# MCG-NKU/E2FGVI

Hardware: AMD Instinct MI355X
Metric: inpainted frames/sec at 432x240 T=10 (higher is better)
Workload: dtype f32; 1 GPU; BASELINE.json configs[1]: e2fgvi 432x240 T=10 l_t=10, 1 clip(s) per GPU per forward (1 in the job), random-init weights, torch.rand frames + box mask (SURVEY.md 8d); clips_per_gpu=1, precision=fp32, kernel_selection=e2fgvi_amd/tile_table.py (checked in, deterministic: ops.py), hip_graph=True, forwards_in_flight=2

## Files before the change

### e2fgvi_amd/build.py

```python
import os
import subprocess
import sys
from concurrent.futures import ThreadPoolExecutor

HERE = os.path.dirname(os.path.abspath(__file__))
CSRC = os.path.join(HERE, "csrc")
LIB = os.path.join(CSRC, "libe2fgvi_hip.so")
FLAGS = ["--offload-arch=gfx950", "-O3", "-std=c++17", "-fPIC", "-ffp-contract=fast"]
NOPK = ["-Xclang", "-target-feature", "-Xclang", "-packed-fp32-ops"]
UNITS = [("error.hip", "error.o", []), ("conv.hip", "conv.o", []), ("conv.hip", "conv_nopk.o", NOPK + ["-DE2_NOPK_VARIANT"]),
         ("conv_bf16x.hip", "conv_bf16x.o", NOPK), ("conv_wino.hip", "conv_wino.o", NOPK), ("conv_wino.hip", "conv_wino_x3.o", NOPK + ["-DE2_WINO_X3=1"]), ("conv_wino4.hip", "conv_wino4.o", NOPK), ("conv_tail.hip", "conv_tail.o", NOPK),
         ("mdcn.hip", "mdcn.o", NOPK), ("attention.hip", "attention.o", []),
         ("attention_bf16.hip", "attention_bf16.o", NOPK), ("attention_x3.hip", "attention_x3.o", NOPK), ("misc.hip", "misc.o", NOPK),
         ("video.hip", "video.o", NOPK), ("metrics.hip", "metrics.o", NOPK)]
NOPK_OBJECTS = ("conv_nopk.o", "conv_bf16x.o", "conv_wino.o", "conv_wino4.o", "conv_wino_x3.o", "conv_tail.o", "mdcn.o", "attention_bf16.o", "attention_x3.o", "misc.o", "video.o", "metrics.o")
OBJDUMP = "/opt/rocm/lib/llvm/bin/llvm-objdump"


def _hipcc():
    for c in (os.environ.get("HIPCC"), "/opt/rocm/bin/hipcc"):
        if c and os.path.exists(c):
            return c
    return "hipcc"


def _stale(out, deps):
    return (not os.path.exists(out)) or any(os.path.getmtime(d) > os.path.getmtime(out) for d in deps)


def build(force=False, verbose=False, nopk_all=False, lib=None, tag=None, defines=()):
    hipcc = _hipcc()
    if tag:
        nopk_all = False
    objdir = os.path.join(CSRC, ("build_" + tag) if tag else ("build_nopk" if nopk_all else "build"))
    os.makedirs(objdir, exist_ok=True)
    out = lib or (os.path.join(CSRC, "libe2fgvi_hip_%s.so" % tag) if tag else
                  os.path.join(CSRC, "libe2fgvi_hip_nopk.so") if nopk_all else LIB)
    headers = [os.path.join(CSRC, "common.h"), os.path.join(HERE, "..", "include", "e2fgvi_hip.h"), os.path.abspath(__file__)]
    jobs = []
    for src, obj, extra in UNITS:
        sp, op = os.path.join(CSRC, src), os.path.join(objdir, obj)
        if nopk_all and not any(f == "-packed-fp32-ops" for f in extra):
            extra = extra + NOPK
        if force or _stale(op, [sp] + headers):
            jobs.append([hipcc] + FLAGS + extra + list(defines) + ["-c", sp, "-o", op])

    def run(cmd):
        if verbose:
            print(" ".join(cmd), flush=True)
        subprocess.check_call(cmd)

    with ThreadPoolExecutor(max_workers=min(4, max(1, len(jobs)))) as ex:
        list(ex.map(run, jobs))
    objs = [os.path.join(objdir, obj) for _, obj, _ in UNITS]
    if force or jobs or _stale(out, objs):
        run([hipcc, "--offload-arch=gfx950", "-shared", "-fPIC", "-o", out] + objs)
    if jobs:
        verify_isa(objdir)
        if not nopk_all:
            verify_wino_waits(objdir)
            verify_exit_reuse(objdir)
            verify_no_scratch(objdir)
    return out


def build_variant(tag, *defines):
    return build(tag=tag, defines=defines)


def device_isa(obj):
    import shutil
    import tempfile
    d = tempfile.mkdtemp(prefix="e2isa")
    try:
        local = os.path.join(d, os.path.basename(obj))
        shutil.copy(obj, local)
        subprocess.run([OBJDUMP, "--offloading", os.path.basename(obj)], cwd=d, check=True, stdout=subprocess.DEVNULL,
                       stderr=subprocess.DEVNULL)
        dev = [f for f in os.listdir(d) if "gfx950" in f]
        if not dev:
            return ""
        return subprocess.run([OBJDUMP, "-d", os.path.join(d, dev[0])], check=True, capture_output=True, text=True).stdout
    finally:
        shutil.rmtree(d, ignore_errors=True)


def verify_isa(objdir=None):
    import re
    objdir = objdir or os.path.join(CSRC, "build")
    if not os.path.exists(OBJDUMP):
        return
    for obj in NOPK_OBJECTS:
        isa = device_isa(os.path.join(objdir, obj))
        bad = re.findall(r"v_pk_(?:mul|add|fma)_f32", isa)
        if bad or not isa:
            raise RuntimeError("%s: %s" % (obj, "%d packed-fp32 instructions in a unit that must have none" % len(bad) if isa
                                           else "no gfx950 code object found"))


def verify_no_scratch(objdir=None, obj="conv_bf16x.o", marker="ELb0ELi2ELb1EEE"):
    import re
    import shutil
    import tempfile
    objdir = objdir or os.path.join(CSRC, "build")
    readelf = os.path.join(os.path.dirname(OBJDUMP), "llvm-readelf")
    if not (os.path.exists(OBJDUMP) and os.path.exists(readelf)):
        return 0
    d = tempfile.mkdtemp(prefix="e2elf")
    try:
        shutil.copy(os.path.join(objdir, obj), os.path.join(d, obj))
        subprocess.run([OBJDUMP, "--offloading", obj], cwd=d, check=True, stdout=subprocess.DEVNULL, stderr=subprocess.DEVNULL)
        dev = [f for f in os.listdir(d) if "gfx950" in f]
        notes = subprocess.run([readelf, "--notes", os.path.join(d, dev[0])], check=True, capture_output=True, text=True).stdout if dev else ""
    finally:
        shutil.rmtree(d, ignore_errors=True)
    found = 0
    for block in notes.split("  - .agpr_count")[1:]:
        name = re.search(r"\.name:\s+(\S+)", block)
        if not name or marker not in name.group(1):
            continue
        found += 1
        priv = int(re.search(r"\.private_segment_fixed_size:\s+(\d+)", block).group(1))
        spill = int(re.search(r"\.vgpr_spill_count:\s+(\d+)", block).group(1))
        if priv or spill:
            raise RuntimeError("%s: %s: private segment %d bytes, %d spilled VGPRs in a ping-pong kernel" % (obj, name.group(1)[:70], priv, spill))
    if not found:
        raise RuntimeError("verify_no_scratch: no ping-pong instantiation found in %s (mangled-name marker changed?)" % obj)
    return found


def _kernels(isa):
    import re
    out, cur = {}, None
    for line in isa.splitlines():
        m = re.match(r"^[0-9a-f]+ <([^>]+)>:", line)
        if m:
            cur = out.setdefault(m.group(1), [])
            continue
        m = re.match(r"^\s+(\S+)\s*(.*?)\s*//\s*([0-9A-Fa-f]+):", line)
        if m and cur is not None:
            cur.append((int(m.group(3), 16), m.group(1), m.group(2)))
    return out


def check_kernel_waits(obj, name, ins):
    import re
    vmem = re.compile(r"^(buffer|global|flat|scratch)_(load|store|atomic)")
    marks = [i for i in range(len(ins) - 1) if ins[i][1] == "s_waitcnt" and ins[i + 1][1] == "s_waitcnt"
             and ins[i][2] == ins[i + 1][2] and "vmcnt" in ins[i][2]]
    if not marks:
        return 0
    addr_to_idx = {a: i for i, (a, _, _) in enumerate(ins)}
    spans = []
    for i, (a, mn, ops_) in enumerate(ins):
        if mn.startswith("s_cbranch") or mn == "s_branch":
            try:
                off = int(ops_.split()[0])
            except (ValueError, IndexError):
                continue
            if off >= 32768:
                off -= 65536
            tgt = a + 4 + 4 * off
            if off < 0 and tgt in addr_to_idx:
                spans.append((addr_to_idx[tgt], i))
    loops = 0
    rolling = "conv_wino_x3w_kernel" in name
    for lo, hi in spans:
        inner = [m for m in marks if lo <= m <= hi]
        if not inner or any(lo <= l2 and h2 <= hi and (l2, h2) != (lo, hi) and any(l2 <= m <= h2 for m in inner)
                            for l2, h2 in spans):
            continue
        loops += 1
        if rolling:
            counts = [int(re.search(r"vmcnt\((\d+)\)", ins[m][2]).group(1)) for m in inner]
            for a, b in zip(inner, inner[1:]):
                if any(vmem.match(ins[k][1]) for k in range(a + 2, b)):
                    raise RuntimeError("%s: %s: vector-memory instruction between the group waits at 0x%x and 0x%x"
                                       % (obj, name[:60], ins[a][0], ins[b][0]))
            g = counts[0] - counts[1] if len(counts) > 1 else counts[0]
            if counts[-1] != 0 or g <= 0 or any(c != counts[0] - j * g for j, c in enumerate(counts)):
                raise RuntimeError("%s: %s: group waits %s are not (P-1) G, ..., G, 0" % (obj, name[:60], counts))
            tail = [k for k in list(range(inner[-1] + 2, hi + 1)) + list(range(lo, inner[0])) if vmem.match(ins[k][1])]
            planes = tail[-(counts[0] + g):]
            if len(planes) != counts[0] + g or any(ins[k][1] != "buffer_load_dwordx4" or " lds" in ins[k][2] for k in planes):
                raise RuntimeError("%s: %s: the %d vector-memory instructions in front of the group waits are not the plane "
                                   "loads" % (obj, name[:60], counts[0] + g))
            continue
        for j, m in enumerate(inner):
            n = int(re.search(r"vmcnt\((\d+)\)", ins[m][2]).group(1))
            if j:
                rng = range(inner[j - 1] + 2, m)
            else:
                rng = list(range(inner[-1] + 2, hi + 1)) + list(range(lo, m))
            cnt = sum(1 for k in rng if vmem.match(ins[k][1]))
            if cnt != n:
                raise RuntimeError("%s: %s: explicit s_waitcnt vmcnt(%d) at 0x%x follows %d vector-memory instructions "
                                   "since the previous explicit wait" % (obj, name[:60], n, ins[m][0], cnt))
    return loops


def verify_wino_waits(objdir=None, objects=("conv_wino.o", "conv_wino_x3.o", "conv_wino4.o")):
    objdir = objdir or os.path.join(CSRC, "build")
    if not os.path.exists(OBJDUMP):
        return 0
    loops = 0
    for obj in objects:
        for name, ins in _kernels(device_isa(os.path.join(objdir, obj))).items():
            loops += check_kernel_waits(obj, name, ins)
    if not loops:
        raise RuntimeError("verify_wino_waits: no K loop with marked waits found (disassembly format changed?)")
    return loops


def _vregs(text):
    import re
    r = set()
    for m in re.finditer(r"\bv\[(\d+):(\d+)\]", text):
        r.update(range(int(m.group(1)), int(m.group(2)) + 1))
    for m in re.finditer(r"\bv(\d+)\b", text):
        r.add(int(m.group(1)))
    return r


def _successors(ins, at):
    succ = []
    for i, (a, m, o) in enumerate(ins):
        if m in ("s_endpgm", "s_endpgm_saved"):
            succ.append(())
        elif m == "s_branch" or m.startswith("s_cbranch"):
            off = int(o.split()[0])
            off -= 65536 if off > 32767 else 0
            tgt = at.get(a + 4 + 4 * off)
            if tgt is None:
                raise RuntimeError("branch at 0x%x leaves the kernel" % a)
            succ.append((tgt,) if m == "s_branch" else (tgt, i + 1))
        elif m.startswith("s_setpc") or m.startswith("s_swappc"):
            raise RuntimeError("indirect jump at 0x%x: control flow cannot be followed" % a)
        else:
            succ.append((i + 1,) if i + 1 < len(ins) else ())
    return succ


def check_exit_reuse(obj, name, ins, min_mfma=8):
    import re
    at = {a: i for i, (a, _, _) in enumerate(ins)}
    succ = _successors(ins, at)
    is_mfma = [("mfma" in m) for _, m, _ in ins]
    breg = set()
    for (_, m, o), f in zip(ins, is_mfma):
        if f:
            breg |= _vregs([x.strip() for x in o.split(",")][2])
    wregs = set()
    for _, m, o in ins:
        if re.match(r"buffer_load_dword", m) and not o.rstrip().endswith(" lds"):
            d = _vregs(o.split(",")[0])
            if d & breg:
                wregs |= d
    if not wregs:
        return 0
    n = len(ins)
    index, low, comp = [-1] * n, [0] * n, [-1] * n
    stack, onstack, counter, ncomp = [], [False] * n, 0, 0
    for root in range(n):
        if index[root] >= 0:
            continue
        work = [(root, 0)]
        while work:
            v, pi = work.pop()
            if pi == 0:
                index[v] = low[v] = counter
                counter += 1
                stack.append(v)
                onstack[v] = True
            recurse = False
            for j in range(pi, len(succ[v])):
                w = succ[v][j]
                if index[w] < 0:
                    work.append((v, j + 1))
                    work.append((w, 0))
                    recurse = True
                    break
                if onstack[w]:
                    low[v] = min(low[v], index[w])
            if recurse:
                continue
            if low[v] == index[v]:
                while True:
                    w = stack.pop()
                    onstack[w] = False
                    comp[w] = ncomp
                    if w == v:
                        break
                ncomp += 1
            if work:
                u = work[-1][0]
                low[u] = min(low[u], low[v])
    members = {}
    for k in range(n):
        members.setdefault(comp[k], []).append(k)
    loops = [m for m in members.values() if len(m) > 1 and sum(1 for k in m if is_mfma[k]) >= min_mfma]
    inside = [False] * n
    for m in loops:
        for k in m:
            inside[k] = True
    edges = 0
    for m in loops:
        mine = set(m)
        starts = set()
        for k in m:
            for t in succ[k]:
                if t not in mine:
                    starts.add(t)
        for st in sorted(starts):
            edges += 1
            seen, todo = set(), [(st, False)]
            while todo:
                k, dead = todo.pop()
                if (k, dead) in seen:
                    continue
                seen.add((k, dead))
                a, m, o = ins[k]
                if m == "s_waitcnt" and "vmcnt(0)" in o:
                    continue
                if m.startswith("s_endpgm") or (inside[k] and not dead):
                    raise RuntimeError("%s: %s: the path from the K-loop exit at 0x%x reaches 0x%x (%s) without an s_waitcnt vmcnt(0): "
                                       "weight loads may still be in flight" % (obj, name[:60], ins[st][0], a,
                                                                                "another K loop" if inside[k] else m))
                if not dead and not m.startswith("s_") and _vregs(o) & wregs:
                    raise RuntimeError("%s: %s: 0x%x %s %s touches a register of a weight load that may still be in flight behind the "
                                       "K loop left at 0x%x (no vmcnt(0) yet)" % (obj, name[:60], a, m, o, ins[st][0]))
                flip = m == "s_andn2_saveexec_b64" or (m == "s_xor_b64" and o.startswith("exec"))
                if flip and not dead:
                    dead = True
                elif m in ("s_or_b64", "s_mov_b64") and o.startswith("exec"):
                    dead = False
                nxt = succ[k]
                if dead and m == "s_cbranch_execz":
                    nxt = nxt[:1]
                elif dead and m == "s_cbranch_execnz":
                    nxt = nxt[1:]
                todo.extend((t, dead) for t in nxt)
    return edges


EXIT_REUSE_OBJECTS = ("conv_wino.o", "conv_wino_x3.o", "conv_wino4.o")


def verify_exit_reuse(objdir=None, objects=EXIT_REUSE_OBJECTS):
    objdir = objdir or os.path.join(CSRC, "build")
    if not os.path.exists(OBJDUMP):
        return 0
    n = 0
    for obj in objects:
        for name, ins in _kernels(device_isa(os.path.join(objdir, obj))).items():
            if "conv_wino" not in name or "pack_" in name:
                continue
            k = check_exit_reuse(obj, name, ins)
            if not k:
                raise RuntimeError("verify_exit_reuse: no K-loop exit found in %s: %s (disassembly format changed?)" % (obj, name[:60]))
            n += k
    if not n:
        raise RuntimeError("verify_exit_reuse: no Winograd kernel found")
    return n


if __name__ == "__main__":
    print(build(force="--force" in sys.argv, verbose=True, nopk_all="--nopk-all" in sys.argv))
```

### e2fgvi_amd/csrc/conv_wino4.hip

```cpp
#include "common.h"
#include <utility>

#ifndef E2_CLAIM_AFTER_LOOP
#define E2_CLAIM_AFTER_LOOP(r) asm volatile("" : "+v"(r))
#endif

namespace {

struct W4Params {
    const float* src[E2FGVI_MAX_SRC];
    int ld[E2FGVI_MAX_SRC];
    int coff[E2FGVI_MAX_SRC];
    int cpg[E2FGVI_MAX_SRC];
    unsigned src_bytes[E2FGVI_MAX_SRC];
    int nsrc;
    int N, H, W;
    int Cout, Cout_g, Npad;
    int blocksY, blocksX, tilesN, nblk;
    int nchunks;
    unsigned wgroup_bytes;
    long long wgroup_elems;
    const float* w;
    const float* bias;
    const float* res;
    int res_ld, res_coff;
    float* dst;
    int dst_ld, dst_coff;
    int act;
    float slope;
    int vec_store;
};

__host__ __device__ constexpr float bt4(int r, int c) {
    return r == 0   ? (c == 0 ? 4.f : c == 2 ? -5.f : c == 4 ? 1.f : 0.f)
           : r == 1 ? (c == 1 ? -4.f : c == 2 ? -4.f : c == 3 ? 1.f : c == 4 ? 1.f : 0.f)
           : r == 2 ? (c == 1 ? 4.f : c == 2 ? -4.f : c == 3 ? -1.f : c == 4 ? 1.f : 0.f)
           : r == 3 ? (c == 1 ? -2.f : c == 2 ? -1.f : c == 3 ? 2.f : c == 4 ? 1.f : 0.f)
           : r == 4 ? (c == 1 ? 2.f : c == 2 ? -1.f : c == 3 ? -2.f : c == 4 ? 1.f : 0.f)
                    : (c == 1 ? 4.f : c == 3 ? -5.f : c == 5 ? 1.f : 0.f);
}
__host__ __device__ constexpr float bt2(int r, int c) {
    return r == 0   ? (c == 0 ? 1.f : c == 2 ? -1.f : 0.f)
           : r == 1 ? (c == 1 ? 1.f : c == 2 ? 1.f : 0.f)
           : r == 2 ? (c == 1 ? -1.f : c == 2 ? 1.f : 0.f)
                    : (c == 1 ? 1.f : c == 3 ? -1.f : 0.f);
}
__host__ __device__ constexpr float at4(int r, int c) {
    return r == 0   ? (c < 5 ? 1.f : 0.f)
           : r == 1 ? (c == 1 ? 1.f : c == 2 ? -1.f : c == 3 ? 2.f : c == 4 ? -2.f : 0.f)
           : r == 2 ? (c == 1 ? 1.f : c == 2 ? 1.f : c == 3 ? 4.f : c == 4 ? 4.f : 0.f)
                    : (c == 1 ? 1.f : c == 2 ? -1.f : c == 3 ? 8.f : c == 4 ? -8.f : c == 5 ? 1.f : 0.f);
}
__host__ __device__ constexpr float at2(int r, int c) {
    return r == 0 ? (c < 3 ? 1.f : 0.f) : (c == 1 ? 1.f : c == 2 ? -1.f : c == 3 ? -1.f : 0.f);
}
__host__ __device__ constexpr float g4(int r, int c) {
    return r == 0   ? (c == 0 ? 0.25f : 0.f)
           : r == 1 ? (-1.f / 6.f)
           : r == 2 ? (c == 1 ? 1.f / 6.f : -1.f / 6.f)
           : r == 3 ? (c == 0 ? 1.f / 24.f : c == 1 ? 1.f / 12.f : 1.f / 6.f)
           : r == 4 ? (c == 0 ? 1.f / 24.f : c == 1 ? -1.f / 12.f : 1.f / 6.f)
                    : (c == 2 ? 1.f : 0.f);
}
__host__ __device__ constexpr float g2(int r, int c) {
    return r == 0 ? (c == 0 ? 1.f : 0.f) : r == 1 ? 0.5f : r == 2 ? (c == 1 ? -0.5f : 0.5f) : (c == 2 ? 1.f : 0.f);
}
template <int FY> __host__ __device__ constexpr float bty(int r, int c) { return FY == 2 ? bt2(r, c) : bt4(r, c); }
template <int FY> __host__ __device__ constexpr float aty(int r, int c) { return FY == 2 ? at2(r, c) : at4(r, c); }
__host__ __device__ constexpr float gy(int fy, int r, int c) { return fy == 2 ? g2(r, c) : g4(r, c); }

__device__ __forceinline__ float w4_dcn_post(float v, int co, int C, const float* fl, float max_residue) {
    const int noff = (C / 3) * 2;
    if (co >= noff) return e2_fast_sigmoid(v);
    const int which = (co * 2 >= noff) ? 2 : 0;
    return max_residue * e2_fast_tanh(v) + fl[which + ((co & 1) ? 0 : 1)];
}
__device__ __forceinline__ float w4_act(float v, int act, float slope) {
    if (act == E2FGVI_ACT_RELU) return fmaxf(v, 0.f);
    if (act == E2FGVI_ACT_LRELU) return v > 0.f ? v : v * slope;
    if (act == E2FGVI_ACT_TANH) return tanhf(v);
    return v;
}

__device__ __forceinline__ __amdgpu_buffer_rsrc_t w4_rsrc(const void* base, unsigned bytes) {
    return __builtin_amdgcn_make_buffer_rsrc(const_cast<void*>(base), 0, (int)bytes, 0x00020000);
}
__device__ __forceinline__ f32x4 w4_load4(__amdgpu_buffer_rsrc_t r, unsigned byte_off) {
    return __builtin_bit_cast(f32x4, __builtin_amdgcn_raw_buffer_load_b128(r, (int)byte_off, 0, 0));
}

constexpr int W4_RAW_W = 18;
constexpr unsigned W4_OOB = 0xFFFFFFFFu;
template <int V> struct IC4 { static constexpr int value = V; };
template <class F, int... Is>
__device__ __forceinline__ void w4_static_for_impl(F&& f, std::integer_sequence<int, Is...>) { (f(IC4<Is>{}), ...); }
template <int N, class F>
__device__ __forceinline__ void w4_static_for(F&& f) { w4_static_for_impl(f, std::make_integer_sequence<int, N>{}); }

typedef int w4_i32x4 __attribute__((ext_vector_type(4)));
__device__ __forceinline__ w4_i32x4 w4_rsrc_words(const void* base, unsigned bytes) {
    const unsigned long long b = (unsigned long long)base;
    w4_i32x4 r;
    r[0] = __builtin_amdgcn_readfirstlane((int)(unsigned)b);
    r[1] = __builtin_amdgcn_readfirstlane((int)((unsigned)(b >> 32) & 0xFFFFu));
    r[2] = __builtin_amdgcn_readfirstlane((int)bytes);
    r[3] = 0x00020000;
    return r;
}
__device__ __forceinline__ void w4_load4_pinned(f32x4& v, w4_i32x4 rsrc, unsigned byte_off) {
    asm volatile("buffer_load_dwordx4 %0, %1, %2, 0 offen" : "=v"(v) : "v"(byte_off), "s"(rsrc) : "memory");
}
template <int N>
__device__ __forceinline__ void w4_wait_vmcnt() {
    asm volatile("s_waitcnt vmcnt(%0)\n\ts_waitcnt vmcnt(%0)" ::"n"(N) : "memory");
}

template <int FY, int BN, int SC>
__global__ __launch_bounds__(128 * (FY + 2), 2) void conv_wino4_kernel(const W4Params p) {
    static_assert(FY == 2, "row tile: F(2x4,3x3)");
    static_assert(SC == 2, "chunks per LDS stage (the weight double buffer alternates with the chunk parity)");
    constexpr int NW = 2 * (FY + 2);
    constexpr int NT = 64 * NW;
    constexpr int TN = BN / 32;
    constexpr int NPOS = (FY + 2) * 6;
    constexpr int BH = 8 * FY;
    constexpr int RAW_H = BH + 2;
    constexpr int PLANE_ROW = (FY == 2) ? 6 : 5;
    constexpr int PLANE_RAW = RAW_H * PLANE_ROW * 16;
    constexpr int PLANE_BYTES = PLANE_RAW + ((16 - PLANE_RAW % 128) + 128) % 128;
    static_assert(PLANE_BYTES % 128 == 16, "plane pitch");
    constexpr int CHUNK_BYTES = 8 * PLANE_BYTES;
    constexpr int STAGE_BYTES = SC * CHUNK_BYTES;
    constexpr int EPI_BYTES = NPOS * 16 * 32 * 4;
    constexpr int SMEM = (2 * STAGE_BYTES > EPI_BYTES) ? 2 * STAGE_BYTES : EPI_BYTES;
    constexpr int RAW_ITEMS = RAW_H * W4_RAW_W * 2;
    constexpr int RAW_IT = (RAW_ITEMS + NT - 1) / NT;
    static_assert(NT >= 128 * FY, "epilogue items");

    __shared__ __attribute__((aligned(16))) unsigned char smem[SMEM];

    const int tid = threadIdx.x;
    const int lane = tid & 63, wave = tid >> 6;
    const int g = blockIdx.y;
    const int logical = xcd_remap(blockIdx.x, p.nblk);
    const int mblocks = p.N * p.blocksY * p.blocksX;
    const int tile_n = logical / mblocks;
    int rem = logical - tile_n * mblocks;
    const int img = rem / (p.blocksY * p.blocksX);
    rem -= img * (p.blocksY * p.blocksX);
    const int by = rem / p.blocksX, bx = rem - by * p.blocksX;
    const int n0 = tile_n * BN;
    const int y0 = by * BH - 1, x0 = bx * 16 - 1;

    unsigned raw_off[RAW_IT];
    int raw_dst[RAW_IT];
#pragma unroll
    for (int it = 0; it < RAW_IT; ++it) {
        const int item = tid + it * NT;
        const int kq = item & 1, px = item >> 1;
        const int py = px / W4_RAW_W, pxx = px - py * W4_RAW_W;
        const int gy_ = y0 + py, gx_ = x0 + pxx;
        const bool have = item < RAW_ITEMS;
        const bool in = have && gy_ >= 0 && gy_ < p.H && gx_ >= 0 && gx_ < p.W;
        raw_off[it] = in ? (unsigned)((img * p.H + gy_) * p.W + gx_) : W4_OOB;
        raw_dst[it] = have ? (kq * 4 + (pxx & 3)) * PLANE_BYTES + (py * PLANE_ROW + (pxx >> 2)) * 16 : -1;
    }
    const unsigned raw_kq16 = (unsigned)(tid & 1) * 16u;

    int s = 0, c0 = 0;
    const float* cur_src = p.src[0];
    unsigned cur_bytes = p.src_bytes[0];
    unsigned cur_ld4 = (unsigned)p.ld[0] * 4u;
    unsigned cur_chan = (unsigned)(p.coff[0] + g * p.cpg[0]) * 4u;
    int cur_cpg = p.cpg[0];
    int raw_left = p.nchunks;
    f32x4 rraw[SC][RAW_IT];
    auto load_raw = [&](f32x4 (&q)[RAW_IT]) {
        const __amdgpu_buffer_rsrc_t arsrc = w4_rsrc(cur_src, cur_bytes);
        const unsigned chan = cur_chan + (unsigned)c0 * 4u + raw_kq16;
        const bool cvalid = raw_left-- > 0 && c0 + (int)(raw_kq16 >> 2) < cur_cpg;
#pragma unroll
        for (int it = 0; it < RAW_IT; ++it) {
            unsigned off = (cvalid && raw_off[it] != W4_OOB) ? raw_off[it] * cur_ld4 + chan : W4_OOB;
            asm volatile("" : "+v"(off));
            q[it] = w4_load4(arsrc, off);
        }
        c0 += 8;
        if (c0 >= cur_cpg) {
            c0 = 0;
            ++s;
            if (s == p.nsrc) s = 0;
            if (p.nsrc > 1) {
                cur_src = p.src[s]; cur_bytes = p.src_bytes[s]; cur_ld4 = (unsigned)p.ld[s] * 4u;
                cur_chan = (unsigned)(p.coff[s] + g * p.cpg[s]) * 4u; cur_cpg = p.cpg[s];
            }
        }
    };
    auto store_raw = [&](int buf) {
        unsigned char* base = smem + buf * STAGE_BYTES;
#pragma unroll
        for (int q = 0; q < SC; ++q)
#pragma unroll
            for (int it = 0; it < RAW_IT; ++it)
                if (raw_dst[it] >= 0) *reinterpret_cast<f32x4*>(base + q * CHUNK_BYTES + raw_dst[it]) = rraw[q][it];
    };

    const int xi = wave >> 1, half = wave & 1;
    const int i = lane & 31, h = lane >> 5;
    const int ty = i >> 2, tx = i & 3;
    const int lane_base = (h * 4) * PLANE_BYTES + ((FY * ty) * PLANE_ROW + tx) * 16;

    const w4_i32x4 wrsrc = w4_rsrc_words(p.w + (long long)g * p.wgroup_elems, p.wgroup_bytes);
    const unsigned u_step = (unsigned)(NPOS * 2) * (unsigned)p.Npad * 16u;
    unsigned u_off[3][TN];
#pragma unroll
    for (int a = 0; a < 3; ++a)
#pragma unroll
        for (int n = 0; n < TN; ++n) {
            const int col = n0 + n * 32 + i;
            const int pos = xi * 6 + 3 * half + a;
            u_off[a][n] = col < p.Npad ? (unsigned)(((pos * 2 + h) * p.Npad + col) * 16) : 0x80000000u;
        }
    f32x4 bq[2][3][TN];
    auto load_b = [&](int chunk, f32x4 (&q)[3][TN]) {
#pragma unroll
        for (int a = 0; a < 3; ++a)
#pragma unroll
            for (int n = 0; n < TN; ++n) w4_load4_pinned(q[a][n], wrsrc, u_off[a][n] + (unsigned)chunk * u_step);
    };
    auto claim_b = [&](auto LATER_, f32x4 (&q)[3][TN]) {
        w4_wait_vmcnt<decltype(LATER_)::value>();
#pragma unroll
        for (int a = 0; a < 3; ++a)
#pragma unroll
            for (int n = 0; n < TN; ++n) asm volatile("" : "+v"(q[a][n]));
    };

    f32x16 acc[3][TN];
#pragma unroll
    for (int a = 0; a < 3; ++a)
#pragma unroll
        for (int n = 0; n < TN; ++n)
#pragma unroll
            for (int r = 0; r < 16; ++r) acc[a][n][r] = 0.f;

    const int nstages = (p.nchunks + SC - 1) / SC;
#pragma unroll
    for (int q = 0; q < SC; ++q) load_raw(rraw[q]);
    load_b(0, bq[0]);
    store_raw(0);
#pragma unroll
    for (int q = 0; q < SC; ++q) load_raw(rraw[q]);
    __syncthreads();

    auto k_loop = [&](auto XI_, auto HF_) {
        constexpr int XI = decltype(XI_)::value;
        constexpr int HF = decltype(HF_)::value;
        auto read_col = [&](const unsigned char* raw, f32x4 (&d)[FY + 2], auto J_) {
            constexpr int col = HF + decltype(J_)::value;
#pragma unroll
            for (int r = 0; r < FY + 2; ++r)
                if (bty<FY>(XI, r) != 0.f)
                    d[r] = *reinterpret_cast<const f32x4*>(raw + (col & 3) * PLANE_BYTES + (r * PLANE_ROW + (col >> 2)) * 16);
        };
        auto row_comb = [&](const f32x4 (&d)[FY + 2]) -> f32x4 {
            bool first = true;
            f32x4 acc_e = {0.f, 0.f, 0.f, 0.f};
#pragma unroll
            for (int r = 0; r < FY + 2; ++r) {
                const float c = bty<FY>(XI, r);
                if (c == 0.f) continue;
                acc_e = first ? c * d[r] : acc_e + c * d[r];
                first = false;
            }
            return acc_e;
        };
        auto col_comb = [&](const f32x4 (&e)[5], auto A_) -> f32x4 {
            constexpr int nu = 3 * HF + decltype(A_)::value;
            bool first = true;
            f32x4 acc_v = {0.f, 0.f, 0.f, 0.f};
#pragma unroll
            for (int j = 0; j < 5; ++j) {
                const float c = bt4(nu, HF + j);
                if (c == 0.f) continue;
                acc_v = first ? c * e[j] : acc_v + c * e[j];
                first = false;
            }
            return acc_v;
        };
        for (int st = 0; st < nstages; ++st) {
            const unsigned char* stage = smem + (st & 1) * STAGE_BYTES + lane_base;
#pragma unroll
            for (int q = 0; q < SC; ++q) {
                load_b(SC * st + q + 1, bq[(q & 1) ^ 1]);
                if (q == 0) claim_b(IC4<3 * TN + SC * RAW_IT>{}, bq[q & 1]);
                else claim_b(IC4<3 * TN>{}, bq[q & 1]);
                __builtin_amdgcn_sched_barrier(0);
                const unsigned char* raw = stage + q * CHUNK_BYTES;
                f32x4 d[5][FY + 2];
                f32x4 e[5];
                f32x4 v[3];
                w4_static_for<5>([&](auto J_) { read_col(raw, d[decltype(J_)::value], J_); });
                w4_static_for<5>([&](auto J_) { e[decltype(J_)::value] = row_comb(d[decltype(J_)::value]); });
                v[0] = col_comb(e, IC4<0>{}); v[1] = col_comb(e, IC4<1>{}); v[2] = col_comb(e, IC4<2>{});
#pragma unroll
                for (int k = 0; k < 4; ++k)
#pragma unroll
                    for (int n = 0; n < TN; ++n)
#pragma unroll
                        for (int a = 0; a < 3; ++a)
                            acc[a][n] = __builtin_amdgcn_mfma_f32_32x32x2f32(v[a][k], bq[q & 1][a][n][k], acc[a][n], 0, 0, 0);
            }
            store_raw((st & 1) ^ 1);
#pragma unroll
            for (int q = 0; q < SC; ++q) load_raw(rraw[q]);
            __syncthreads();
        }
        __syncthreads();
    };
    switch (wave) {
        case 0: k_loop(IC4<0>{}, IC4<0>{}); break;
        case 1: k_loop(IC4<0>{}, IC4<1>{}); break;
        case 2: k_loop(IC4<1>{}, IC4<0>{}); break;
        case 3: k_loop(IC4<1>{}, IC4<1>{}); break;
        case 4: k_loop(IC4<2>{}, IC4<0>{}); break;
        case 5: k_loop(IC4<2>{}, IC4<1>{}); break;
        case 6: k_loop(IC4<3>{}, IC4<0>{}); break;
        case 7: k_loop(IC4<3>{}, IC4<1>{}); break;
        default: break;
    }
    asm volatile("s_waitcnt vmcnt(0)" ::: "memory");
#pragma unroll
    for (int b_ = 0; b_ < 2; ++b_)
#pragma unroll
        for (int a = 0; a < 3; ++a)
#pragma unroll
            for (int n = 0; n < TN; ++n) E2_CLAIM_AFTER_LOOP(bq[b_][a][n]);

    float* E = reinterpret_cast<float*>(smem);
    const int HW = p.H * p.W;
    const int pos0 = xi * 6 + 3 * half;
#pragma unroll
    for (int nh = 0; nh < TN; ++nh) {
#pragma unroll
        for (int th = 0; th < 2; ++th) {
            if (nh || th) __syncthreads();
#pragma unroll
            for (int a = 0; a < 3; ++a)
#pragma unroll
                for (int rr = 0; rr < 8; ++rr) {
                    const int r = th * 8 + rr;
                    const int lt = (rr & 3) + 8 * (rr >> 2) + 4 * h;
                    E[((pos0 + a) * 16 + lt) * 32 + i] = acc[a][nh][r];
                }
            __syncthreads();
            const int cq = tid & 7, lt = (tid >> 3) & 15, oy = tid >> 7;
            const int tile = 16 * th + lt;
            const int n = n0 + nh * 32 + cq * 4;
            const int oyy = by * BH + FY * (tile >> 2) + oy, oxx = bx * 16 + 4 * (tile & 3);
            if (tid < 128 * FY && n < p.Cout_g && oyy < p.H && oxx < p.W) {
                f32x4 sc[6];
#pragma unroll
                for (int nu = 0; nu < 6; ++nu) sc[nu] = f32x4{0.f, 0.f, 0.f, 0.f};
#pragma unroll
                for (int x = 0; x < FY + 2; ++x) {
                    float cy = 0.f;
#pragma unroll
                    for (int o = 0; o < FY; ++o) cy = (oy == o) ? aty<FY>(o, x) : cy;
#pragma unroll
                    for (int nu = 0; nu < 6; ++nu) {
                        const f32x4 m = *reinterpret_cast<const f32x4*>(E + ((x * 6 + nu) * 16 + lt) * 32 + cq * 4);
                        sc[nu] = sc[nu] + cy * m;
                    }
                }
                f32x4 y[4];
#pragma unroll
                for (int ox = 0; ox < 4; ++ox) {
                    bool first = true;
                    f32x4 a4 = {0.f, 0.f, 0.f, 0.f};
#pragma unroll
                    for (int nu = 0; nu < 6; ++nu) {
                        const float c = at4(ox, nu);
                        if (c == 0.f) continue;
                        a4 = first ? c * sc[nu] : a4 + c * sc[nu];
                        first = false;
                    }
                    y[ox] = a4;
                }
                const int co = g * p.Cout_g + n;
                const long long pix0 = (long long)img * HW + (long long)oyy * p.W + oxx;
                const bool full = n + 3 < p.Cout_g;
                f32x4 bv = {0.f, 0.f, 0.f, 0.f};
                if (p.bias) {
#pragma unroll
                    for (int c = 0; c < 4; ++c) bv[c] = (full || n + c < p.Cout_g) ? p.bias[co + c] : 0.f;
                }
#pragma unroll
                for (int px = 0; px < 4; ++px) {
                    const long long pix = pix0 + px;
                    f32x4 v = y[px] + bv;
                    if (p.act == E2FGVI_ACT_DCNPOST) {
                        const f32x4 fl = *reinterpret_cast<const f32x4*>(p.res + pix * 4);
                        const float flv[4] = {fl[0], fl[1], fl[2], fl[3]};
#pragma unroll
                        for (int c = 0; c < 4; ++c) v[c] = w4_dcn_post(v[c], co + c, p.Cout, flv, p.slope);
                    } else {
                        if (p.res) {
                            const float* r = p.res + pix * p.res_ld + p.res_coff + co;
                            if (p.vec_store && full) v = v + *reinterpret_cast<const f32x4*>(r);
                            else {
#pragma unroll
                                for (int c = 0; c < 4; ++c) if (full || n + c < p.Cout_g) v[c] += r[c];
                            }
                        }
#pragma unroll
                        for (int c = 0; c < 4; ++c) v[c] = w4_act(v[c], p.act, p.slope);
                    }
                    float* o = p.dst + pix * p.dst_ld + p.dst_coff + co;
                    if (p.vec_store && full) *reinterpret_cast<f32x4*>(o) = v;
                    else {
#pragma unroll
                        for (int c = 0; c < 4; ++c) if (full || n + c < p.Cout_g) o[c] = v[c];
                    }
                }
            }
        }
    }
}

struct W4Pack {
    int Cout, groups, nsrc, fy, npos;
    int cpg[E2FGVI_MAX_SRC];
    int Cout_g, Npad, Cin_g, nchunks;
    long long wgroup_elems, total;
};

bool w4_geometry(int Cout, int groups, int nsrc, const int32_t* cpg, int fy, W4Pack* q) {
    if (Cout <= 0 || groups <= 0 || Cout % groups || nsrc < 1 || nsrc > E2FGVI_MAX_SRC || fy != 2) return false;
    q->Cout = Cout; q->groups = groups; q->nsrc = nsrc; q->fy = fy; q->npos = (fy + 2) * 6;
    q->Cout_g = Cout / groups;
    q->Npad = round_up(q->Cout_g, 32);
    q->Cin_g = 0; q->nchunks = 0;
    for (int s = 0; s < E2FGVI_MAX_SRC; ++s) q->cpg[s] = 0;
    for (int s = 0; s < nsrc; ++s) {
        if (cpg[s] <= 0 || cpg[s] % 4) return false;
        q->cpg[s] = cpg[s];
        q->Cin_g += cpg[s];
        q->nchunks += (cpg[s] + 7) / 8;
    }
    q->wgroup_elems = (long long)q->nchunks * q->npos * 2 * q->Npad * 4;
    q->total = q->wgroup_elems * groups;
    return true;
}

__global__ void pack_wino4_weight_kernel(const float* __restrict__ w, float* __restrict__ wp, const W4Pack p) {
    const long long idx = (long long)blockIdx.x * blockDim.x + threadIdx.x;
    if (idx >= p.total) return;
    const int g = (int)(idx / p.wgroup_elems);
    long long rem = idx - (long long)g * p.wgroup_elems;
    const int kk = (int)(rem & 3);
    rem >>= 2;
    const int n = (int)(rem % p.Npad);
    rem /= p.Npad;
    const int kq = (int)(rem & 1);
    rem >>= 1;
    const int a = (int)(rem % p.npos);
    const int chunk = (int)(rem / p.npos);
    int s = 0, prefix = 0, lc = chunk;
    while (lc >= (p.cpg[s] + 7) / 8) { lc -= (p.cpg[s] + 7) / 8; prefix += p.cpg[s]; ++s; }
    const int ch = lc * 8 + kq * 4 + kk;
    float v = 0.f;
    if (n < p.Cout_g && ch < p.cpg[s]) {
        const float* f = w + ((long long)(g * p.Cout_g + n) * p.Cin_g + prefix + ch) * 9;
        const int xi = a / 6, nu = a - xi * 6;
        float acc = 0.f;
        for (int r = 0; r < 3; ++r) {
            const float gr = gy(p.fy, xi, r);
            float row = 0.f;
            for (int c = 0; c < 3; ++c) row += f[r * 3 + c] * g4(nu, c);
            acc += gr * row;
        }
        v = acc;
    }
    wp[idx] = v;
}

template <int FY, int BN>
int launch_wino4(W4Params& p, int groups, hipStream_t st) {
    p.blocksY = cdiv(p.H, 8 * FY);
    p.blocksX = cdiv(p.W, 16);
    p.tilesN = cdiv(p.Cout_g, BN);
    const long long nblk = (long long)p.N * p.blocksY * p.blocksX * p.tilesN;
    E2_REQUIRE(nblk < 2147483647LL, E2FGVI_EUNSUP, "conv3x3_winograd4: grid too large");
    p.nblk = (int)nblk;
    hipLaunchKernelGGL((conv_wino4_kernel<FY, BN, 2>), dim3(p.nblk, groups, 1), dim3(128 * (FY + 2)), 0, st, p);
    E2_LAUNCH_CHECK("conv3x3_winograd4");
    return 0;
}

}

extern "C" int64_t e2fgvi_packed_winograd4_weight_size(int32_t Cout, int32_t groups, int32_t nsrc, const int32_t* src_cpg,
                                                       int32_t fy) {
    W4Pack q;
    if (!src_cpg || !w4_geometry(Cout, groups, nsrc, src_cpg, fy, &q)) {
        e2fgvi_set_error("packed_winograd4_weight_size: bad geometry (channels per source multiples of 4, fy = 2)");
        return E2FGVI_EINVAL;
    }
    return q.total;
}

extern "C" int e2fgvi_pack_winograd4_weight(const float* w, float* wpacked, int32_t Cout, int32_t groups, int32_t nsrc,
                                            const int32_t* src_cpg, int32_t fy, void* stream) {
    W4Pack q;
    E2_REQUIRE(w && wpacked && src_cpg, E2FGVI_EINVAL, "pack_winograd4_weight: null pointer");
    E2_REQUIRE(w4_geometry(Cout, groups, nsrc, src_cpg, fy, &q), E2FGVI_EINVAL, "pack_winograd4_weight: bad geometry");
    hipLaunchKernelGGL(pack_wino4_weight_kernel, dim3((unsigned)cdiv64(q.total, 256)), dim3(256), 0, (hipStream_t)stream, w,
                       wpacked, q);
    E2_LAUNCH_CHECK("pack_winograd4_weight");
    return 0;
}

extern "C" int e2fgvi_conv3x3_winograd4(const e2fgvi_conv_desc* d, int32_t fy, void* stream) {
    E2_REQUIRE(d, E2FGVI_EINVAL, "conv3x3_winograd4: null descriptor");
    W4Pack q;
    E2_REQUIRE(w4_geometry(d->Cout, d->groups, d->nsrc, d->src_cpg, fy, &q), E2FGVI_EINVAL,
               "conv3x3_winograd4: bad geometry (channels per source must be multiples of 4, fy = 2)");
    E2_REQUIRE(d->KH == 3 && d->KW == 3 && d->stride == 1 && d->pad == 1, E2FGVI_EUNSUP,
               "conv3x3_winograd4: only 3x3, stride 1, pad 1");
    E2_REQUIRE(d->N > 0 && d->H > 0 && d->W > 0 && d->H % fy == 0 && d->W % 4 == 0, E2FGVI_EUNSUP,
               "conv3x3_winograd4: H must be a multiple of fy and W a multiple of 4");
    E2_REQUIRE(d->Ho == d->H && d->Wo == d->W, E2FGVI_EINVAL, "conv3x3_winograd4: Ho/Wo must equal H/W");
    E2_REQUIRE(d->wpacked && d->dst, E2FGVI_EINVAL, "conv3x3_winograd4: null weight/dst");
    E2_REQUIRE(!d->dst_nchw, E2FGVI_EUNSUP, "conv3x3_winograd4: NCHW output not supported");
    E2_REQUIRE(d->dst_coff >= 0 && d->dst_coff + d->Cout <= d->dst_ld, E2FGVI_EINVAL, "conv3x3_winograd4: dst slice exceeds dst_ld");
    if (d->act == E2FGVI_ACT_DCNPOST)
        E2_REQUIRE(d->residual && d->Cout % 3 == 0 && d->groups == 1 && ((uintptr_t)d->residual & 15) == 0, E2FGVI_EINVAL,
                   "conv3x3_winograd4: ACT_DCNPOST needs the [pixel][4] flows as residual, Cout %% 3 == 0, groups == 1");
    W4Params p;
    for (int s = 0; s < E2FGVI_MAX_SRC; ++s) { p.src[s] = nullptr; p.ld[s] = 0; p.coff[s] = 0; p.cpg[s] = 0; p.src_bytes[s] = 0; }
    for (int s = 0; s < d->nsrc; ++s) {
        E2_REQUIRE(d->src[s], E2FGVI_EINVAL, "conv3x3_winograd4: null source %d", s);
        E2_REQUIRE(d->src_ld[s] % 4 == 0 && d->src_coff[s] % 4 == 0 && ((uintptr_t)d->src[s] & 15) == 0, E2FGVI_EINVAL,
                   "conv3x3_winograd4: source %d not 16-byte addressable", s);
        E2_REQUIRE(d->src_coff[s] + d->groups * d->src_cpg[s] <= d->src_ld[s], E2FGVI_EINVAL,
                   "conv3x3_winograd4: source %d channel range exceeds its pixel stride", s);
        const long long bytes = (long long)d->N * d->H * d->W * d->src_ld[s] * 4;
        E2_REQUIRE(bytes < 4294967295LL, E2FGVI_EUNSUP, "conv3x3_winograd4: source %d spans >= 4 GiB (split the batch)", s);
        p.src[s] = d->src[s]; p.ld[s] = d->src_ld[s]; p.coff[s] = d->src_coff[s]; p.cpg[s] = d->src_cpg[s];
        p.src_bytes[s] = (unsigned)bytes;
    }
    E2_REQUIRE(q.wgroup_elems * 4 < 0x70000000LL, E2FGVI_EUNSUP, "conv3x3_winograd4: packed weight group >= 1.75 GiB");
    E2_REQUIRE(((uintptr_t)d->wpacked & 15) == 0, E2FGVI_EINVAL, "conv3x3_winograd4: packed weight not 16-byte aligned");
    p.nsrc = d->nsrc;
    p.N = d->N; p.H = d->H; p.W = d->W;
    p.Cout = d->Cout; p.Cout_g = q.Cout_g; p.Npad = q.Npad;
    p.nchunks = q.nchunks;
    p.wgroup_elems = q.wgroup_elems; p.wgroup_bytes = (unsigned)(q.wgroup_elems * 4);
    p.w = (const float*)d->wpacked; p.bias = d->bias;
    p.res = d->residual; p.res_ld = d->res_ld; p.res_coff = d->res_coff;
    p.dst = d->dst; p.dst_ld = d->dst_ld; p.dst_coff = d->dst_coff;
    p.act = d->act; p.slope = d->slope;
    bool vec = ((uintptr_t)d->dst & 15) == 0 && d->dst_ld % 4 == 0 && d->dst_coff % 4 == 0 && q.Cout_g % 4 == 0;
    if (d->residual && d->act != E2FGVI_ACT_DCNPOST)
        vec = vec && ((uintptr_t)d->residual & 15) == 0 && d->res_ld % 4 == 0 && d->res_coff % 4 == 0;
    p.vec_store = vec ? 1 : 0;
    hipStream_t st = (hipStream_t)stream;
    int tile = d->tile;
    if (!tile) tile = 64;
    if (fy == 2 && tile == 64) return launch_wino4<2, 64>(p, d->groups, st);
    e2fgvi_set_error("conv3x3_winograd4: fy must be 2 and tile 0 (auto) or 64 couts per workgroup (the other shapes were pruned in round 6)");
    return E2FGVI_EUNSUP;
}
```

### e2fgvi_amd/lib.py

```python
import ctypes as C
import os

_HERE = os.path.dirname(os.path.abspath(__file__))
LIB_PATH = os.environ.get("E2FGVI_LIB") or os.path.join(_HERE, "csrc", "libe2fgvi_hip.so")

ABI_VERSION = 9
MAX_SRC = 4
ACT_NONE, ACT_RELU, ACT_LRELU, ACT_TANH, ACT_DCNPOST = 0, 1, 2, 3, 4
DT_F32, DT_BF16 = 0, 1
DT_BF16X3 = 2
DT_F16 = 3

_fp = C.c_void_p


class ConvDesc(C.Structure):
    _fields_ = [
        ("src", _fp * MAX_SRC), ("src_ld", C.c_int32 * MAX_SRC), ("src_coff", C.c_int32 * MAX_SRC),
        ("src_cpg", C.c_int32 * MAX_SRC), ("nsrc", C.c_int32),
        ("N", C.c_int32), ("H", C.c_int32), ("W", C.c_int32), ("Ho", C.c_int32), ("Wo", C.c_int32),
        ("KH", C.c_int32), ("KW", C.c_int32), ("stride", C.c_int32), ("pad", C.c_int32),
        ("groups", C.c_int32), ("Cout", C.c_int32), ("bk", C.c_int32),
        ("wpacked", _fp), ("bias", _fp), ("residual", _fp), ("res_ld", C.c_int32), ("res_coff", C.c_int32),
        ("dst", _fp), ("dst_ld", C.c_int32), ("dst_coff", C.c_int32), ("dst_nchw", C.c_int32),
        ("act", C.c_int32), ("slope", C.c_float), ("tile", C.c_int32),
    ]


class ConvXDesc(C.Structure):
    _fields_ = [
        ("src", _fp * MAX_SRC), ("src_ld", C.c_int32 * MAX_SRC), ("src_coff", C.c_int32 * MAX_SRC),
        ("src_cpg", C.c_int32 * MAX_SRC), ("nsrc", C.c_int32),
        ("N", C.c_int32), ("H", C.c_int32), ("W", C.c_int32), ("Ho", C.c_int32), ("Wo", C.c_int32),
        ("KH", C.c_int32), ("KW", C.c_int32), ("stride", C.c_int32), ("pad", C.c_int32),
        ("groups", C.c_int32), ("Cout", C.c_int32),
        ("wpacked", _fp), ("bias", _fp), ("residual", _fp), ("res_ld", C.c_int32), ("res_coff", C.c_int32),
        ("res_dtype", C.c_int32),
        ("dst", _fp), ("dst_ld", C.c_int32), ("dst_coff", C.c_int32), ("dst_dtype", C.c_int32),
        ("dst2", _fp), ("dst2_ld", C.c_int32), ("dst2_coff", C.c_int32),
        ("act", C.c_int32), ("slope", C.c_float), ("tile", C.c_int32), ("dst_nchw", C.c_int32), ("tap_packed", C.c_int32),
        ("out_grid", C.c_int32), ("pad_left", C.c_int32),
        ("out_sy", C.c_int32), ("out_sx", C.c_int32), ("out_py", C.c_int32), ("out_px", C.c_int32),
        ("out_H", C.c_int32), ("out_W", C.c_int32), ("res_bcast", C.c_int32),
        ("dst2_split_from", C.c_int32), ("dst2_plane_stride", C.c_int64),
    ]


class MdcnDesc(C.Structure):
    _fields_ = [
        ("src", _fp * 2), ("src_ld", C.c_int32 * 2), ("src_c", C.c_int32 * 2), ("nsrc", C.c_int32),
        ("N", C.c_int32), ("H", C.c_int32), ("W", C.c_int32), ("Ho", C.c_int32), ("Wo", C.c_int32),
        ("KH", C.c_int32), ("KW", C.c_int32), ("stride", C.c_int32), ("pad", C.c_int32), ("dil", C.c_int32),
        ("deform_groups", C.c_int32), ("Cout", C.c_int32),
        ("offset", _fp), ("off_ld", C.c_int32), ("mask", _fp), ("mask_ld", C.c_int32),
        ("flows", _fp), ("max_residue", C.c_float),
        ("wpacked", _fp), ("bias", _fp),
        ("dst", _fp), ("dst_ld", C.c_int32), ("dst_coff", C.c_int32), ("tile", C.c_int32), ("dst_dtype", C.c_int32),
        ("mfma_dtype", C.c_int32), ("src_dtype", C.c_int32), ("src_planar", C.c_int32),
    ]


_i32, _i64, _f = C.c_int32, C.c_int64, C.c_float
SYMBOLS = {
    "e2fgvi_last_error": (C.c_char_p, []),
    "e2fgvi_abi_version": (C.c_int, []),
    "e2fgvi_nhwc_to_planar16": (C.c_int, [_fp, _fp, _i64, _i32, _fp]),
    "e2fgvi_conv2d_nhwc": (C.c_int, [C.POINTER(ConvDesc), _fp]),
    "e2fgvi_conv2d_nhwc_nopk": (C.c_int, [C.POINTER(ConvDesc), _fp]),
    "e2fgvi_conv2d_x": (C.c_int, [C.POINTER(ConvXDesc), _i32, _fp]),
    "e2fgvi_packed_conv_weight_x_size": (_i64, [_i32, _i32, _i32, _i32, _i32, _i32, _i32, C.POINTER(_i32)]),
    "e2fgvi_pack_conv_weight_x": (C.c_int, [_fp, _fp, _i32, _i32, _i32, _i32, _i32, _i32, _i32, C.POINTER(_i32), _fp]),
    "e2fgvi_packed_conv_weight_size": (_i64, [_i32, _i32, _i32, _i32, _i32, C.POINTER(_i32), _i32]),
    "e2fgvi_pack_conv_weight": (C.c_int, [_fp, _fp, _i32, _i32, _i32, _i32, _i32, C.POINTER(_i32), _i32, _fp]),
    "e2fgvi_packed_winograd_weight_size": (_i64, [_i32, _i32, _i32, C.POINTER(_i32)]),
    "e2fgvi_pack_winograd_weight": (C.c_int, [_fp, _fp, _i32, _i32, _i32, C.POINTER(_i32), _fp]),
    "e2fgvi_conv3x3_winograd": (C.c_int, [C.POINTER(ConvDesc), _fp]),
    "e2fgvi_packed_winograd_weight_x3_size": (_i64, [_i32, _i32, _i32, C.POINTER(_i32)]),
    "e2fgvi_pack_winograd_weight_x3": (C.c_int, [_fp, _fp, _i32, _i32, _i32, C.POINTER(_i32), _fp]),
    "e2fgvi_conv3x3_winograd_x3": (C.c_int, [C.POINTER(ConvDesc), _fp]),
    "e2fgvi_packed_winograd4_weight_size": (_i64, [_i32, _i32, _i32, C.POINTER(_i32), _i32]),
    "e2fgvi_pack_winograd4_weight": (C.c_int, [_fp, _fp, _i32, _i32, _i32, C.POINTER(_i32), _i32, _fp]),
    "e2fgvi_conv3x3_winograd4": (C.c_int, [C.POINTER(ConvDesc), _i32, _fp]),
    "e2fgvi_packed_tail_weight_size": (_i64, [_i32, _i32]),
    "e2fgvi_pack_tail_weight": (C.c_int, [_fp, _fp, _i32, _i32, _i32, _fp]),
    "e2fgvi_conv3x3_tail": (C.c_int, [_fp, _i32, _i32, _fp, _fp, _fp, _i32, _i32, _i32, _i32, C.c_float, _fp]),
    "e2fgvi_mdcn_nhwc": (C.c_int, [C.POINTER(MdcnDesc), _fp]),
    "e2fgvi_packed_dcn_weight_size": (_i64, [_i32, _i32, _i32, _i32, _i32]),
    "e2fgvi_pack_dcn_weight": (C.c_int, [_fp, _fp, _i32, _i32, _i32, _i32, _i32, _i32, _fp]),
    "e2fgvi_focal_attention": (C.c_int, [_fp, _fp, _fp, _i32, _fp, _fp, _i32, _i32, _i32, _i32, _i32, _fp]),
    "e2fgvi_split3_kv": (C.c_int, [_fp, _fp, _i64, _fp]),
    "e2fgvi_focal_attention_x3": (C.c_int, [_fp, _fp, _fp, _i32, _fp, _fp, _i32, _i32, _i32, _i32, _i32, _fp]),
    "e2fgvi_nchw_to_nhwc": (C.c_int, [_fp, _fp, _i32, _i32, _i32, _i32, _i32, _i32, _f, _f, _fp]),
    "e2fgvi_nhwc_to_nchw": (C.c_int, [_fp, _i32, _fp, _i32, _i32, _i32, _i32, _fp]),
    "e2fgvi_resize_bilinear": (C.c_int, [_fp, _i32, _i32, _i32, _fp, _i32, _i32, _i32, _i32, _i32, _i32, _i32, _i32, _fp, _fp, _fp]),
    "e2fgvi_avgpool2_nhwc": (C.c_int, [_fp, _fp, _i32, _i32, _i32, _i32, _fp]),
    "e2fgvi_spynet_level_input": (C.c_int, [_fp, _fp, _fp, _fp, _fp, _fp, _i32, _i32, _i32, _i32, _fp]),
    "e2fgvi_prop_cond": (C.c_int, [_fp, _i32, _fp, _i32, _i32, _fp, _fp, _i64, _fp, _i32, _fp, _fp, _i32, _i32, _i32, _i32, _fp]),
    "e2fgvi_layernorm": (C.c_int, [_fp, _fp, _fp, _fp, _i32, _i64, _i32, _fp]),
    "e2fgvi_window_pool": (C.c_int, [_fp, _i32, _fp, _fp, _fp, _i32, _i32, _i32, _i32, _fp]),
    "e2fgvi_ffn_fold": (C.c_int, [_fp, _fp, _i32, _i32, _i32, _i32, _i32, _i32, _i32, _i32, _fp]),
    "e2fgvi_ffn_unfold": (C.c_int, [_fp, _fp, _i32, _i32, _i32, _i32, _i32, _i32, _i32, _i32, _fp]),
    "e2fgvi_mask_prepare": (C.c_int, [_fp, _i32, _i32, _i32, _fp, _fp, _fp, _i32, _i32, _i32, _fp]),
    "e2fgvi_masked_clip": (C.c_int, [_fp, _fp, _fp, _i32, _i32, _i32, _fp, _i32, _i32, _fp]),
    "e2fgvi_composite": (C.c_int, [_fp, _fp, _fp, _i32, _fp, _fp, _fp, _i32, _i32, _i32, _i32, _fp]),
    "e2fgvi_resample_u8": (C.c_int, [_fp, _fp, _i32, _i32, _i32, _i32, _i32, _fp, _fp, _i32, _fp]),
    "e2fgvi_restore_u8": (C.c_int, [_fp, _fp, _fp, _fp, _i32, _i32, _i32, _i32, _i32, _fp, _fp, _fp, _fp, _i32, _fp, _fp, _i32, _fp]),
    "e2fgvi_float_to_u8": (C.c_int, [_fp, _fp, _i64, _fp]),
    "e2fgvi_pred_to_u8": (C.c_int, [_fp, _fp, _i32, _i32, _i32, _i32, _i32, _fp]),
    "e2fgvi_gather_slabs": (C.c_int, [_fp, _i32, _fp, _i32, _i64, _fp, _fp]),
    "e2fgvi_scatter_slabs": (C.c_int, [_fp, _fp, _i32, _i64, _fp, _i32, _fp]),
    "e2fgvi_psnr_ssim_workspace": (_i64, [_i32, _i32, _i32]),
    "e2fgvi_psnr_ssim": (C.c_int, [_fp, _fp, _i32, _i32, _i32, _i32, _fp, _fp, _fp]),
    "e2fgvi_softcomp_fold": (C.c_int, [_fp, _fp, _fp, _fp, _i32, _i32, _i32, _i32, _i32, _i32, _i32, _fp]),
    "e2fgvi_focal_attention_16": (C.c_int, [_fp, _fp, _fp, _i32, _fp, _fp, _i32, _i32, _i32, _i32, _i32, _fp]),
    "e2fgvi_focal_attention_16_variant": (C.c_int, [C.c_int]),
    "e2fgvi_cast": (C.c_int, [_fp, _i32, _fp, _i32, _i64, _fp]),
}

_lib = None

TRACE = None
NEXT_META = None


X3_PIPE = 6 * 157.3 / 2500.0


def useful_macs(kernel, macs, issued):
    import re
    k = str(kernel)
    f = 1.0
    m = re.match(r"conv_wino4<F\((\d)x4\)", k)
    if m:
        fy = int(m.group(1))
        f = (fy + 2) * 6 / (fy * 4 * 9.0)
    elif k.startswith("conv_wino"):
        f = 16 / 36.0
    if "x3" in k:
        f *= X3_PIPE
    return min(int(issued), int(macs * f))


def annotate(**meta):
    global NEXT_META
    if TRACE is not None:
        if "macs" in meta and "issued" in meta and "useful" not in meta:
            meta["useful"] = useful_macs(meta.get("kernel", ""), meta["macs"], meta["issued"])
        NEXT_META = meta


def _traced(name, fn):
    def call(*args):
        global NEXT_META
        if TRACE is None:
            return fn(*args)
        import torch
        e0, e1 = torch.cuda.Event(enable_timing=True), torch.cuda.Event(enable_timing=True)
        e0.record()
        rc = fn(*args)
        e1.record()
        if name.startswith("e2fgvi_pack_"):
            TRACE.append({"symbol": name, "e0": e0, "e1": e1, "meta": None})
            return rc
        TRACE.append({"symbol": name, "e0": e0, "e1": e1, "meta": NEXT_META})
        NEXT_META = None
        return rc
    call.__name__ = name
    return call


class HipLibraryMissing(ImportError):
    pass


def load():
    global _lib
    if _lib is not None:
        return _lib
    if not os.path.exists(LIB_PATH):
        raise HipLibraryMissing(
            "libe2fgvi_hip.so not found at %s -- the MI355X kernels are mandatory (no CPU / eager "
            "fallback exists).  Build them: python -m e2fgvi_amd.build" % LIB_PATH)
    lib = C.CDLL(LIB_PATH)
    for name, (res, args) in SYMBOLS.items():
        try:
            fn = getattr(lib, name)
        except AttributeError:
            raise HipLibraryMissing("%s does not export %s: rebuild it (python -m e2fgvi_amd.build)" % (LIB_PATH, name)) from None
        fn.restype = res
        fn.argtypes = args
        if args and args[-1] is _fp and res is C.c_int:
            setattr(lib, name, _traced(name, fn))
    have = int(lib.e2fgvi_abi_version())
    if have != ABI_VERSION:
        raise HipLibraryMissing("%s implements ABI version %d, this binding is version %d: rebuild it (python -m e2fgvi_amd.build)"
                                % (LIB_PATH, have, ABI_VERSION))
    _lib = lib
    return lib


class HipError(RuntimeError):
    pass


def library_key():
    import hashlib
    try:
        with open(LIB_PATH, "rb") as fh:
            return hashlib.sha256(fh.read()).hexdigest()[:16]
    except OSError:
        return None


def check(rc, what):
    if rc != 0:
        msg = load().e2fgvi_last_error()
        raise HipError("%s failed (code %d): %s" % (what, rc, msg.decode() if msg else "?"))
```

### e2fgvi_amd/ops.py

```python
import collections
import ctypes as C
import math
import os

import torch

from . import lib as _L

ACT_NONE, ACT_RELU, ACT_LRELU, ACT_TANH, ACT_DCNPOST = _L.ACT_NONE, _L.ACT_RELU, _L.ACT_LRELU, _L.ACT_TANH, _L.ACT_DCNPOST


def _stream():
    return C.c_void_p(torch.cuda.current_stream().cuda_stream)


def _chk(t, name, dtype=torch.float32):
    if not isinstance(t, torch.Tensor) or not t.is_cuda:
        raise TypeError("%s must be a CUDA (ROCm) tensor -- the HIP path has no CPU fallback" % name)
    if t.dtype != dtype:
        raise TypeError("%s must be %s, got %s" % (name, dtype, t.dtype))
    if not t.is_contiguous():
        raise ValueError("%s must be contiguous" % name)
    return t


def _ptr(t):
    return C.c_void_p(t.data_ptr()) if t is not None else C.c_void_p(0)


def empty_nhwc(n, h, w, c, device):
    return torch.empty((n, h, w, c), dtype=torch.float32, device=device)


TUNE_CANDIDATES = (0, 213, 223, 211, 219, 216)
WINO_CANDIDATES = (64, 132, 164, 32)
W4_CODES = {2464: (2, 64)}
_W4_MINPIX = 20000
XTUNE_CANDIDATES = (1, 4, 6, 7, 8, 2, 5, 3, 107, 108)
XTUNE_ROWSHIFT = (11, 16, 17, 12, 13, 18)
X3_ENABLED = os.environ.get("E2FGVI_X3", "1") != "0"
X3_MARGIN = 0.97
X3_BASE = 30000
W3_BASE = 40000
W3_CANDIDATES = (132, 164, 32, 5132, 6064)
W3_WIDE = 6064
W3_WIDE_FALLBACK = 164
DMA_BASE = 2000


def _decode(code):
    if code >= W3_BASE:
        return "w3", code - W3_BASE
    if code >= X3_BASE:
        return "x3", code - X3_BASE
    if code in W4_CODES:
        return "w4", code
    if DMA_BASE <= code < DMA_BASE + 100:
        return "dma", code - DMA_BASE
    return "own", code


_TUNED = {}
AUTOTUNE = os.environ.get("E2FGVI_AUTOTUNE", "0") == "1"
TUNE_REPS = max(1, int(os.environ.get("E2FGVI_TUNE_REPS", "1") or 1))
TABLE_FORMAT = 2
_SIZE_FIELD = 8


def _default_tune_file():
    try:
        st = os.stat(_L.LIB_PATH)
        d = os.environ.get("E2FGVI_CACHE_DIR") or os.path.join(os.path.dirname(os.path.abspath(__file__)), ".tile_cache")
        os.makedirs(d, exist_ok=True)
        dev = "gpu"
        if torch.cuda.is_available():
            dev = "".join(ch for ch in torch.cuda.get_device_properties(0).gcnArchName.split(":")[0] if ch.isalnum())
        return os.path.join(d, "tiles_v%d_%s_%x_%x.txt" % (TABLE_FORMAT, dev, st.st_size, int(st.st_mtime)))
    except (OSError, RuntimeError):
        return None


_TUNE_FILE = None
if AUTOTUNE:
    _TUNE_FILE = os.environ.get("E2FGVI_TUNE_FILE")
    if _TUNE_FILE is None:
        _TUNE_FILE = _default_tune_file()
    elif _TUNE_FILE in ("", "0"):
        _TUNE_FILE = None
    if _TUNE_FILE and os.path.exists(_TUNE_FILE):
        import ast
        for _line in open(_TUNE_FILE):
            try:
                _k, _v = ast.literal_eval(_line)
                _TUNED[_k] = _v
            except Exception:
                pass
elif os.environ.get("E2FGVI_TILE_TABLE", "1") != "0":
    try:
        if os.environ.get("E2FGVI_TILE_TABLE", "1").endswith(".py"):
            import importlib.util
            _spec = importlib.util.spec_from_file_location("e2fgvi_tile_table_override", os.environ["E2FGVI_TILE_TABLE"])
            _tt = importlib.util.module_from_spec(_spec)
            _spec.loader.exec_module(_tt)
        else:
            from . import tile_table as _tt
        if getattr(_tt, "TABLE_FORMAT", None) == TABLE_FORMAT:
            _TUNED.update(_tt.TILES)
    except ImportError:
        pass


def _remember(key, tile):
    _TUNED[key] = tile
    if _TUNE_FILE:
        try:
            with open(_TUNE_FILE, "a") as fh:
                fh.write(repr((key, tile)) + "\n")
        except OSError:
            pass
    return tile


def _decision(key):
    best = _TUNED.get(key)
    if best is not None or AUTOTUNE:
        return best
    hit = _NEAREST.get(key)
    if hit is None:
        sc = key[_SIZE_FIELD]
        cands = [(abs(k[_SIZE_FIELD] - sc), k[_SIZE_FIELD], v) for k, v in _TUNED.items()
                 if len(k) == len(key) and k[:_SIZE_FIELD] == key[:_SIZE_FIELD] and k[_SIZE_FIELD + 1:] == key[_SIZE_FIELD + 1:]]
        hit = _NEAREST[key] = (min(cands)[2] if cands else -1)
    return None if hit < 0 else hit


_NEAREST = {}


def sync_tile_decisions(group=None, src=0):
    import torch.distributed as dist
    if not dist.is_available() or not dist.is_initialized() or dist.get_world_size(group) == 1:
        return False
    box = [dict(_TUNED) if dist.get_rank(group) == src else None]
    dist.broadcast_object_list(box, src=src, group=group)
    _TUNED.clear()
    _TUNED.update(box[0])
    _NEAREST.clear()
    return True


def _no_capture(what):
    if torch.cuda.is_available() and torch.cuda.is_current_stream_capturing():
        raise RuntimeError("%s: first use of this kernel's weight packing under HIP-graph capture -- run one eager forward of the "
                           "same shapes before capturing (runner.ShardedStep does)" % what)


_PENDING = []


def _await_pending():
    if torch.cuda.is_current_stream_capturing():
        return
    cur = torch.cuda.current_stream()
    live = []
    for ent in _PENDING:
        sid, ev, waiting = ent
        if ev.query():
            continue
        live.append(ent)
        if sid != cur.cuda_stream and cur.cuda_stream not in waiting:
            cur.wait_event(ev)
            waiting.add(cur.cuda_stream)
    _PENDING[:] = live


def _lazy(store, key, what, build):
    obj = store.get(key)
    if obj is None:
        _no_capture(what)
        obj = store[key] = build()
        if torch.cuda.is_available():
            ev = torch.cuda.Event()
            ev.record()
            _PENDING.append([torch.cuda.current_stream().cuda_stream, ev, set()])
    elif _PENDING:
        _await_pending()
    return obj


def _time_launches(launch, reps):
    e0, e1 = torch.cuda.Event(enable_timing=True), torch.cuda.Event(enable_timing=True)
    e0.record()
    for _ in range(reps):
        launch()
    e1.record()
    e1.synchronize()
    return e0.elapsed_time(e1) / reps


def _pack_weights(size_fn, pack_fn, src, dtype, what, *geom, extra=()):
    n = size_fn(*geom)
    if n < 0:
        _L.check(int(n), "packed_%s_size" % what)
    t = torch.empty(int(n), dtype=dtype, device=src.device)
    _L.check(pack_fn(_ptr(src), _ptr(t), *geom, *extra, _stream()), "pack_" + what)
    return t


def _image_chunks(N, per_img):
    step = max(1, N)
    if N > 1 and N * per_img >= (1 << 32) - 1:
        step = max(1, ((1 << 32) - 2) // per_img)
    for n0 in range(0, N, step):
        yield n0, min(N, n0 + step)


class _ConvLayer:

    def _init_layer(self, weight, bias, cpg, groups, stride, pad):
        if weight.dim() == 2:
            weight = weight[:, :, None, None]
        w = _chk(weight.detach().float().contiguous(), "weight")
        self.Cout, cin_g, self.KH, self.KW = w.shape
        self.cpg = [int(c) for c in cpg]
        if sum(self.cpg) != cin_g:
            raise ValueError("sum(cpg)=%d != weight input channels %d" % (sum(self.cpg), cin_g))
        self.groups, self.stride, self.pad = groups, stride, pad
        self.bias = None if bias is None else _chk(bias.detach().float().contiguous(), "bias")
        self.name = "conv"
        self.tune = False
        self.try_x3 = False
        self.alt3 = None
        return w

    def out_hw(self, H, W):
        return ((H + 2 * self.pad - self.KH) // self.stride + 1, (W + 2 * self.pad - self.KW) // self.stride + 1)

    def _cpg_arr(self):
        return (C.c_int32 * len(self.cpg))(*self.cpg)

    def _srcs_out(self, sources, out, out_nchw, out_dtype):
        srcs = [(s, 0) if isinstance(s, torch.Tensor) else s for s in sources]
        if len(srcs) != len(self.cpg):
            raise ValueError("expected %d sources, got %d" % (len(self.cpg), len(srcs)))
        if out is None:
            N, H, W, _ = srcs[0][0].shape
            Ho, Wo = self.out_hw(H, W)
            out = torch.empty((N, self.Cout, Ho, Wo) if out_nchw else (N, Ho, Wo, self.Cout),
                              dtype=torch.float32 if out_nchw else out_dtype, device=srcs[0][0].device)
        return srcs, out

    def _x_alternative(self, **kw):
        alt = PackedConvX(self._w_raw, self.bias, self.cpg, groups=self.groups, stride=self.stride, pad=self.pad, dtype=torch.float32, **kw)
        alt.name = self.name
        return alt

    def _fill(self, d, src_dtype, chk, srcs, out, out_coff, act, slope, out_nchw):
        N, H, W, _ = srcs[0][0].shape
        Ho, Wo = self.out_hw(H, W)
        for i, (t, coff) in enumerate(srcs):
            _chk(t, "source %d" % i, src_dtype)
            if t.dim() != 4 or tuple(t.shape[:3]) != (N, H, W):
                raise ValueError("source %d shape %s does not match [%d,%d,%d,*]" % (i, tuple(t.shape), N, H, W))
            d.src[i], d.src_ld[i], d.src_coff[i], d.src_cpg[i] = t.data_ptr(), t.shape[3], coff, self.cpg[i]
        d.nsrc = len(srcs)
        d.N, d.H, d.W, d.Ho, d.Wo = N, H, W, Ho, Wo
        d.KH, d.KW, d.stride, d.pad = self.KH, self.KW, self.stride, self.pad
        d.groups, d.Cout = self.groups, self.Cout
        d.bias = self.bias.data_ptr() if self.bias is not None else None
        chk(out, "out")
        if out_nchw:
            if tuple(out.shape) != (N, self.Cout, Ho, Wo) or out.dtype != torch.float32:
                raise ValueError(self._NCHW_ERROR % dict(got=tuple(out.shape), want=(N, self.Cout, Ho, Wo)))
            d.dst_ld, d.dst_coff, d.dst_nchw = 0, 0, 1
        else:
            if out.dim() != 4 or tuple(out.shape[:3]) != (N, Ho, Wo):
                raise ValueError("out shape %s != [%d,%d,%d,*]" % (tuple(out.shape), N, Ho, Wo))
            d.dst_ld, d.dst_coff, d.dst_nchw = out.shape[3], out_coff, 0
        d.dst = out.data_ptr()
        d.act, d.slope, d.tile = act, slope, 0
        return d

    @staticmethod
    def _fill_residual(d, chk, residual, res_coff):
        if residual is not None:
            chk(residual, "residual")
            if residual.dim() != 4 or tuple(residual.shape[:3]) != (d.N, d.Ho, d.Wo):
                raise ValueError("residual shape %s != [%d,%d,%d,*]" % (tuple(residual.shape), d.N, d.Ho, d.Wo))
            d.residual, d.res_ld, d.res_coff = residual.data_ptr(), residual.shape[3], res_coff


_Plan = collections.namedtuple("_Plan", "family tile static from_table use_wino")
_Call = collections.namedtuple("_Call", "d srcs kw kv_planes")


class PackedConv(_ConvLayer):

    _NCHW_ERROR = "NCHW out shape %(got)s != %(want)s"

    def __init__(self, weight, bias, cpg, groups=1, stride=1, pad=0, bk=None, precision="fp32", algo="igemm"):
        lib = _L.load()
        w = self._init_layer(weight, bias, cpg, groups, stride, pad)
        if precision != "fp32":
            raise ValueError("PackedConv is the fp32 layer; the bf16 data path uses PackedConvX")
        self.precision = precision
        self.nopk = False
        self.alt = None
        self._w_raw = w
        if algo not in ("igemm", "winograd", "auto"):
            raise ValueError("algo must be 'igemm', 'winograd' or 'auto'")
        wino_ok = (self.KH, self.KW, stride, pad) == (3, 3, 1, 1) and not any(c % 4 for c in self.cpg)
        if algo == "winograd" and not wino_ok:
            raise ValueError("winograd needs fp32, 3x3 / stride 1 / pad 1 and channels per source in multiples of 4")
        if algo == "auto":
            algo = "auto" if wino_ok else "igemm"
        self.algo = algo
        self._w4 = {}
        self._w3 = None
        self._w_oihw = w if algo in ("winograd", "auto") else None
        self._own = {}
        if algo in ("winograd", "auto"):
            _L.check(min(0, int(lib.e2fgvi_packed_winograd_weight_size(*self._wgeom()))), "packed_winograd_weight_size")
        if algo == "winograd":
            self.bk = 8
            return
        if bk is None:
            pad32 = sum((c + 31) // 32 * 32 for c in self.cpg)
            pad16 = sum((c + 15) // 16 * 16 for c in self.cpg)
            bk = 32 if pad32 <= 1.08 * sum(self.cpg) else (16 if pad16 <= 1.08 * sum(self.cpg) else 8)
        self.bk = bk
        _L.check(min(0, int(lib.e2fgvi_packed_conv_weight_size(self.Cout, groups, self.KH, self.KW, len(self.cpg), self._cpg_arr(), bk))),
                 "packed_conv_weight_size")

    def _wgeom(self):
        return self.Cout, self.groups, len(self.cpg), self._cpg_arr()

    @property
    def wino_packed(self):
        if self.algo not in ("winograd", "auto"):
            return None

        def build():
            lib = _L.load()
            return _pack_weights(lib.e2fgvi_packed_winograd_weight_size, lib.e2fgvi_pack_winograd_weight, self._w_raw, torch.float32,
                                 "winograd_weight", *self._wgeom())
        return _lazy(self._own, "wino", self.name + " (Winograd F(2x2,3x3) weights)", build)

    @property
    def wpacked(self):
        if self.algo == "winograd":
            return None

        def build():
            lib = _L.load()
            return _pack_weights(lib.e2fgvi_packed_conv_weight_size, lib.e2fgvi_pack_conv_weight, self._w_raw, torch.float32,
                                 "conv_weight", self.Cout, self.groups, self.KH, self.KW, len(self.cpg), self._cpg_arr(), self.bk)
        return _lazy(self._own, "igemm", self.name + " (implicit-GEMM weights)", build)

    def weight_bytes(self):
        ts = list(self._own.values()) + list(self._w4.values()) + ([self._w3] if self._w3 is not None else [])
        return sum(t.numel() * t.element_size() for t in ts) + sum(a.weight_bytes() for a in (self.alt, self.alt3) if a is not None)

    def _wino4(self, fy):
        def build():
            lib = _L.load()
            return _pack_weights(lib.e2fgvi_packed_winograd4_weight_size, lib.e2fgvi_pack_winograd4_weight, self._w_oihw, torch.float32,
                                 "winograd4_weight", *self._wgeom(), fy)
        return _lazy(self._w4, fy, self.name + " (Winograd F(%dx4,3x3) weights)" % fy, build)

    def _wino4_rule(self, N, H, W):
        if W % 4 or self._w_oihw is None:
            return 0
        if self.Cout // self.groups >= 256 and sum(self.cpg) >= 256 and N * H * W >= _W4_MINPIX:
            return 2464
        return 0

    def _alt(self):
        return _lazy(vars(self), "alt", self.name + " (LDS-DMA fp32 alternative)", self._x_alternative)

    def _wino_x3(self):
        if self._w_oihw is None:
            return None

        def build():
            lib = _L.load()
            return _pack_weights(lib.e2fgvi_packed_winograd_weight_x3_size, lib.e2fgvi_pack_winograd_weight_x3, self._w_oihw,
                                 torch.bfloat16, "winograd_weight_x3", *self._wgeom())
        return _lazy(vars(self), "_w3", self.name + " (split-operand Winograd weights)", build)

    def _alt3(self):
        if any(c % 4 for c in self.cpg):
            return self.alt3
        return _lazy(vars(self), "alt3", self.name + " (split-operand GEMM alternative)", lambda: self._x_alternative(x3=True))

    def _work(self, d, use_wino, family, tile):
        N, H, W, Ho, Wo = d.N, d.H, d.W, d.Ho, d.Wo
        cin_g, cout_g, K2 = sum(self.cpg), self.Cout // self.groups, self.KH * self.KW
        macs = N * Ho * Wo * self.Cout * cin_g * K2
        asked = int(tile)
        if family == "w4":
            fy, bn = W4_CODES[tile]
            pix = N * (-(-H // (8 * fy)) * 8 * fy) * (-(-W // 16) * 16)
            cin_p = sum(-(-c // 8) * 8 for c in self.cpg)
            issued = pix * (-(-cout_g // bn) * bn) * self.groups * cin_p * (fy + 2) * 6 // (fy * 4)
            kern = "conv_wino4<F(%dx4),%d>" % (fy, bn)
        elif family == "w3":
            asked = W3_BASE + tile
            shape = tile % 1000
            mt, bn = (2, shape) if shape < 100 else (1, shape - 100)
            pix = N * (-(-H // (8 * mt)) * 8 * mt) * (-(-W // 16) * 16)
            cin_p = -(-sum(-(-c // 8) for c in self.cpg) // 2) * 16
            issued = int(pix * (-(-cout_g // bn) * bn) * self.groups * cin_p * 4 * 6 * 157.3 / 2500.0)
            kern = ("conv_wino_x3w<%d>" % bn) if tile >= 6000 else ("conv_wino_x3p4<%d>" % bn) if tile >= 5000 else "conv_wino_x3<%d,%d>" % (mt, bn)
        elif use_wino:
            if not tile:
                big = N * -(-H // 16) * -(-W // 16) * -(-cout_g // 64) * self.groups
                tile = 64 if (cout_g >= 256 and big >= 128) else 132
            mt, bn = (2, tile) if tile < 100 else (1, tile - 100)
            pix = N * (-(-H // (8 * mt)) * 8 * mt) * (-(-W // 16) * 16)
            cin_p = sum(-(-c // 8) * 8 for c in self.cpg)
            issued = pix * (-(-cout_g // bn) * bn) * self.groups * cin_p * 4
            kern = "conv_wino<%d,%d>" % (mt, bn)
        else:
            g = self.bk
            cin_p = sum(-(-c // g) * g for c in self.cpg)
            issued = N * Ho * Wo * (-(-cout_g // 32) * 32) * self.groups * cin_p * K2
            kern = "conv_igemm/halo tile=%d" % tile
        return dict(layer=self.name, kernel=kern, shape="N%d %dx%d %d->%d k%d s%d g%d" % (
            N, H, W, cin_g * self.groups, self.Cout, self.KH, self.stride, self.groups), macs=macs, issued=issued, tile=asked)

    def __call__(self, sources, out=None, out_coff=0, residual=None, res_coff=0, act=ACT_NONE, slope=0.0,
                 out_nchw=False, tile=0, kv_planes=None, out_dtype=None):
        if out_dtype not in (None, torch.float32):
            raise ValueError("PackedConv writes fp32 results")
        srcs, out = self._srcs_out(sources, out, out_nchw, torch.float32)
        N, H, W, _ = srcs[0][0].shape
        kw = dict(out_coff=out_coff, res_coff=res_coff, act=act, slope=slope, out_nchw=out_nchw)
        chunks = list(_image_chunks(N, max(H * W * t.shape[3] * 4 for t, _ in srcs)))
        if len(chunks) > 1:
            for n0, n1 in chunks:
                self([(t[n0:n1], c) for t, c in srcs], out=out[n0:n1], residual=None if residual is None else residual[n0:n1],
                     tile=tile, **kw)
        else:
            kw.update(out=out, residual=residual)
            call = _Call(self._desc(srcs, **kw), srcs, kw, kv_planes)
            if self._launch(call, self._select(call, tile)):
                return out
        if kv_planes is not None:
            split3_kv(out.view(-1, out.shape[-1]), out=kv_planes)
        return out

    def _desc(self, srcs, out, out_coff, residual, res_coff, act, slope, out_nchw):
        d = self._fill(_L.ConvDesc(), torch.float32, _chk, srcs, out, out_coff, act, slope, out_nchw)
        self._fill_residual(d, _chk, residual, res_coff)
        d.bk = self.bk
        return d

    def _select(self, call, tile):
        d, kw = call.d, call.kw
        N, H, W, Ho, Wo = d.N, d.H, d.W, d.Ho, d.Wo
        out, residual = kw["out"], kw["residual"]
        use_wino = self.algo == "winograd" or (self.algo == "auto" and H % 2 == 0 and W % 2 == 0 and not kw["out_nchw"]
                                               and (tile in (0, 32, 64, 132, 164) or _decode(tile)[0] in ("w4", "w3")))
        asked = _decode(tile) if use_wino else ("own", tile)
        static = self._wino4_rule(N, H, W) if use_wino and (tile == 0 or asked[0] == "w3") else tile
        own = ("w4" if use_wino and static in W4_CODES else "own", static)
        family, arg = asked if asked[0] == "w3" else own
        plan = _Plan(family, arg, own, False, use_wino)
        x3 = self.try_x3 and X3_ENABLED
        if not (tile == 0 and (static == 0 or not self.tune) and (self.tune or x3) and N * Ho * Wo >= 2048):
            return plan
        key = (self.Cout, tuple(self.cpg), self.KH, self.KW, self.stride, self.pad, self.groups, self.bk,
               int(4.0 * math.log2(N * Ho * Wo)), residual is not None, kw["act"], use_wino, bool(self.tune), int(static)) + (("x3",) if x3 else ())
        best = _decision(key)
        from_table = best is not None
        if best is None and AUTOTUNE and not torch.cuda.is_current_stream_capturing() and (
                residual is None or residual.data_ptr() != out.data_ptr()):
            best = _remember(key, self._tune(call, own, use_wino, x3))
        family, arg = _decode(best or 0)
        if family in ("w3", "x3") or (self.tune and (family == "dma" or (family == "own" and arg < DMA_BASE))):
            plan = plan._replace(family=family, tile=arg)
        return plan._replace(from_table=from_table)

    def _tune(self, call, own, use_wino, x3):
        d, srcs, kw, kv_planes = call
        best = self._autotune(d, use_wino) if self.tune else own[1]
        base = own if own[0] == "w4" else ("own", best)
        mine = None

        def time_mine():
            self._run(d, *base, use_wino)
            return min(_time_launches(lambda: self._run(d, *base, use_wino), 3) for _ in range(TUNE_REPS))
        if self.tune and not use_wino and not self.nopk:
            alt = self._alt()
            mine = time_mine()
            res = alt._time_tiles(alt._desc(srcs, out2=None, **kw))
            if res and min(res.values()) < mine:
                best, mine = DMA_BASE + min(res, key=res.get), min(res.values())
        if x3 and self._alt3() is not None:
            if mine is None:
                mine = time_mine()
            d3 = self.alt3._desc(srcs, out2=None, **kw)
            if kv_planes is not None:
                self.alt3._set_planes(d3, kv_planes, self.Cout - kv_planes.shape[2], d.N * d.Ho * d.Wo)
            res = self.alt3._time_tiles(d3)
            if res and min(res.values()) < X3_MARGIN * mine:
                best, mine = X3_BASE + min(res, key=res.get), min(res.values())
        if x3 and use_wino and self._wino_x3() is not None:
            w3 = {}
            for shape in W3_CANDIDATES:
                def run():
                    return self._run(d, "w3", shape, use_wino)[0]
                if run() == 0:
                    w3[shape] = min(_time_launches(run, 3) for _ in range(TUNE_REPS))
            if w3 and min(w3.values()) < X3_MARGIN * mine:
                best, mine = W3_BASE + min(w3, key=w3.get), min(w3.values())
        return best

    def _autotune(self, d, wino):
        lib = _L.load()
        best, best_ms = 0, float("inf")
        st = _stream()
        fn = lib.e2fgvi_conv3x3_winograd if wino else lib.e2fgvi_conv2d_nhwc
        d.tile, d.wpacked = 0, (self.wino_packed if wino else self.wpacked).data_ptr()
        for _ in range(3):
            fn(C.byref(d), st)
        for code in (WINO_CANDIDATES if wino else TUNE_CANDIDATES):
            d.tile = code
            if fn(C.byref(d), st) != 0:
                continue
            ms = min(_time_launches(lambda: fn(C.byref(d), st), 2) for _ in range(TUNE_REPS))
            if ms < best_ms:
                best, best_ms = code, ms
        return best

    def _run(self, d, family, tile, use_wino):
        lib, st = _L.load(), _stream()
        if family == "w3":
            d.tile, d.wpacked = tile, self._wino_x3().data_ptr()
            return lib.e2fgvi_conv3x3_winograd_x3(C.byref(d), st), "conv3x3_winograd_x3"
        if family == "w4":
            fy, d.tile = W4_CODES[tile]
            d.wpacked = self._wino4(fy).data_ptr()
            return lib.e2fgvi_conv3x3_winograd4(C.byref(d), fy, st), "conv3x3_winograd4"
        d.tile = tile
        d.wpacked = (self.wino_packed if use_wino else self.wpacked).data_ptr()
        if use_wino:
            return lib.e2fgvi_conv3x3_winograd(C.byref(d), st), "conv3x3_winograd"
        if self.nopk:
            return lib.e2fgvi_conv2d_nhwc_nopk(C.byref(d), st), "conv2d_nhwc_nopk"
        return lib.e2fgvi_conv2d_nhwc(C.byref(d), st), "conv2d_nhwc"

    def _launch(self, call, plan):
        d, srcs, kw, kv_planes = call
        family, tile = plan.family, plan.tile
        try:
            if family == "x3" and self._alt3() is not None:
                self.alt3(srcs, tile=tile, planes=kv_planes, split_from=(self.Cout - kv_planes.shape[2]) if kv_planes is not None else 0,
                          **kw)
                return True
            if family == "dma":
                self._alt()(srcs, tile=tile, **kw)
                return False
            if family == "x3" or (family == "w3" and self._wino_x3() is None):
                family, tile = plan.static
        except _L.HipError:
            if not plan.from_table:
                raise
            family, tile = plan.static
        if _L.TRACE is not None:
            _L.annotate(**self._work(d, plan.use_wino, family, tile))
        rc, what = self._run(d, family, tile, plan.use_wino)
        if rc != 0 and (family, tile) != plan.static:
            rc, what = self._run(d, *plan.static, plan.use_wino)
        _L.check(rc, what)
        return False


HALF16 = (torch.bfloat16, torch.float16)


_DT_CODE = {torch.float32: _L.DT_F32, torch.bfloat16: _L.DT_BF16, torch.float16: _L.DT_F16}


def _dt(t):
    try:
        return _DT_CODE[t.dtype]
    except KeyError:
        raise TypeError("tensor must be float32, bfloat16 or float16, got %s" % t.dtype) from None


def _dt_key(t):
    return _L.DT_BF16 if t.dtype == torch.float16 else _dt(t)


def _chk_any(t, name):
    if not isinstance(t, torch.Tensor) or not t.is_cuda:
        raise TypeError("%s must be a CUDA (ROCm) tensor -- the HIP path has no CPU fallback" % name)
    if not t.is_contiguous():
        raise ValueError("%s must be contiguous" % name)
    _dt(t)
    return t


class PackedConvX(_ConvLayer):

    _NCHW_ERROR = "NCHW out must be fp32 %(want)s"

    def __init__(self, weight, bias, cpg, groups=1, stride=1, pad=0, dtype=torch.bfloat16, taps=None, x3=False):
        lib = _L.load()
        w = self._init_layer(weight, bias, cpg, groups, stride, pad)
        self.dtype = dtype
        self.f32 = dtype == torch.float32
        self.x3 = bool(x3)
        if self.x3 and not self.f32:
            raise ValueError("x3 splitting is for fp32 sources")
        self.f16 = dtype == torch.float16
        if not self.f32 and dtype not in HALF16:
            raise TypeError("PackedConvX: dtype must be float32, bfloat16 or float16")
        self._mode = mode = _L.DT_BF16X3 if self.x3 else _DT_CODE[dtype]
        conv2d_x = lib.e2fgvi_conv2d_x
        self._fn = lambda desc_ref, stream: conv2d_x(desc_ref, mode, stream)
        self._w_raw = w if (self.f32 and not self.x3) else None
        self._taps_arg = taps
        self.taps = (len(self.cpg) == 1 and groups == 1 and self.cpg[0] <= 56 and self.KW > 1
                     and (taps is True if self.f32 else taps is not False))
        self._wdtype = torch.bfloat16 if self.x3 else dtype
        self._wp = None
        if self._w_raw is None:
            self._wp = self._pack(w)
        else:
            _L.check(min(0, int(lib.e2fgvi_packed_conv_weight_x_size(*self._wgeom()))), "packed_conv_weight_x_size")

    @property
    def wpacked(self):
        return _lazy(vars(self), "_wp", self.name + " (LDS-DMA GEMM weights)", lambda: self._pack(self._w_raw))

    def weight_bytes(self):
        return (0 if self._wp is None else self._wp.numel() * self._wp.element_size()) + (self.alt3.weight_bytes() if self.alt3 is not None else 0)

    def _wgeom(self):
        return self._mode, int(self.taps), self.Cout, self.groups, self.KH, self.KW, len(self.cpg), self._cpg_arr()

    def _pack(self, w):
        lib = _L.load()
        return _pack_weights(lib.e2fgvi_packed_conv_weight_x_size, lib.e2fgvi_pack_conv_weight_x, w, self._wdtype, "conv_weight_x",
                             *self._wgeom())

    def _alt3(self):
        if self._w_raw is None:
            return self.alt3
        return _lazy(vars(self), "alt3", self.name + " (split-operand GEMM alternative)",
                     lambda: self._x_alternative(taps=self._taps_arg, x3=True))

    def _desc(self, srcs, out, out_coff, residual, res_coff, act, slope, out2, out_nchw):
        d = self._fill(_L.ConvXDesc(), self.dtype, _chk_any, srcs, out, out_coff, act, slope, out_nchw)
        d.wpacked = None if self._wp is None else self._wp.data_ptr()
        d.dst_dtype = _dt(out)
        if out2 is not None:
            _chk(out2, "out2", torch.float16 if self.f16 else torch.bfloat16)
            if out2.dim() != 4 or tuple(out2.shape[:3]) != (d.N, d.Ho, d.Wo):
                raise ValueError("out2 shape %s != [%d,%d,%d,*]" % (tuple(out2.shape), d.N, d.Ho, d.Wo))
            d.dst2, d.dst2_ld, d.dst2_coff = out2.data_ptr(), out2.shape[3], 0
        self._fill_residual(d, _chk_any, residual, res_coff)
        if residual is not None:
            d.res_dtype = _dt(residual)
        d.tap_packed = 1 if self.taps else 0
        return d

    @staticmethod
    def _set_planes(d, planes, split_from, rows):
        _chk(planes, "planes", torch.bfloat16)
        if planes.dim() != 3 or planes.shape[0] != 3 or planes.shape[1] != rows or planes.shape[2] != d.Cout - split_from:
            raise ValueError("planes must be [3, %d, %d] bf16, got %s" % (rows, d.Cout - split_from, tuple(planes.shape)))
        d.dst2, d.dst2_ld, d.dst2_coff = planes.data_ptr(), planes.shape[2], 0
        d.dst2_split_from, d.dst2_plane_stride = split_from, planes.shape[1] * planes.shape[2]

    def __call__(self, sources, out=None, out_dtype=None, out_coff=0, residual=None, res_coff=0, act=ACT_NONE,
                 slope=0.0, out2=None, tile=0, out_nchw=False, planes=None, split_from=0):
        if out_dtype is None:
            out_dtype = self.dtype
        srcs, out = self._srcs_out(sources, out, out_nchw, out_dtype)
        N, H, W, _ = srcs[0][0].shape
        Ho, Wo = self.out_hw(H, W)
        kw = dict(out_coff=out_coff, res_coff=res_coff, act=act, slope=slope, out_nchw=out_nchw)
        chunks = list(_image_chunks(N, max(H * W * t.shape[3] * (4 if self.f32 else 2) for t, _ in srcs)))
        if len(chunks) > 1:
            if planes is not None:
                raise ValueError("split planes: the batch spans >= 4 GiB (call in chunks)")
            for n0, n1 in chunks:
                self([(t[n0:n1], c) for t, c in srcs], out=out[n0:n1], residual=None if residual is None else residual[n0:n1],
                     out2=None if out2 is None else out2[n0:n1], tile=tile, **kw)
            return out
        kw.update(out=out, residual=residual, out2=out2)
        d = self._desc(srcs, **kw)
        if planes is not None:
            self._set_planes(d, planes, split_from, N * Ho * Wo)
        if tile == 0 and self.tune and N * Ho * Wo >= 2048:
            family, tile = self._select(d, srcs, kw)
            if family == "x3":
                try:
                    return self.alt3(srcs, out_dtype=out_dtype, tile=tile, planes=planes, split_from=split_from, **kw)
                except _L.HipError:
                    tile = 0
        d.tile = tile
        if _L.TRACE is not None:
            _L.annotate(**self._work(d))
        d.wpacked = self.wpacked.data_ptr()
        rc = self._fn(C.byref(d), _stream())
        if rc != 0 and d.tile and self.tune:
            d.tile = 0
            rc = self._fn(C.byref(d), _stream())
        _L.check(rc, "conv2d_x")
        return out

    def _select(self, d, srcs, kw):
        out, residual = kw["out"], kw["residual"]
        x3 = self.try_x3 and X3_ENABLED and self.f32 and not self.x3
        key = (("x3" if self.x3 else ("x32+3" if x3 else "x32")) if self.f32 else "x", self.Cout, tuple(self.cpg), self.KH, self.KW, self.stride, self.pad, self.groups,
               int(4.0 * math.log2(d.N * d.Ho * d.Wo)), _dt_key(out), kw["out_nchw"], self.taps)
        best = _decision(key)
        if best is None and AUTOTUNE and not torch.cuda.is_current_stream_capturing() and (
                residual is None or residual.data_ptr() != out.data_ptr()):
            best = _remember(key, self._tune(d, srcs, kw, x3))
        if _decode(best or 0)[0] in ("x3", "w3"):
            return ("x3", best - X3_BASE) if self._alt3() is not None else ("own", 0)
        return "own", best or 0

    def _tune(self, d, srcs, kw, x3):
        res = self._time_tiles(d)
        best = min(res, key=res.get) if res else 0
        if x3 and self._alt3() is not None:
            res3 = self.alt3._time_tiles(self.alt3._desc(srcs, **kw))
            if res3 and (not res or min(res3.values()) < X3_MARGIN * min(res.values())):
                best = X3_BASE + min(res3, key=res3.get)
        return best

    def _work(self, d):
        N, H, W, Ho, Wo, tile = d.N, d.H, d.W, d.Ho, d.Wo, d.tile
        cin_g, cout_g, K2 = sum(self.cpg), self.Cout // self.groups, self.KH * self.KW
        kc = 32 if self.f32 else 64
        cin_p = sum(-(-c // kc) * kc for c in self.cpg)
        if self.taps:
            cin_p = -(-K2 * (self.cpg[0] // (4 if self.f32 else 8)) // 8) * kc / K2
        return dict(layer=self.name, kernel="conv_%s tile=%d%s" % (("f32x3" if self.x3 else "f32x") if self.f32 else
                                                                   "f16x" if self.f16 else "bf16x", tile, " taps" if self.taps else ""),
                    shape="N%d %dx%d %d->%d k%d s%d g%d" % (N, H, W, cin_g * self.groups, self.Cout, self.KH, self.stride, self.groups),
                    macs=N * Ho * Wo * self.Cout * cin_g * K2, tile=int(tile),
                    issued=int(N * Ho * Wo * (-(-cout_g // 32) * 32) * self.groups * cin_p * K2 * (_L.X3_PIPE if self.x3 else 1)))

    def _time_tiles(self, d, reps=3, rounds=2):
        st = _stream()
        res = {}
        d.tile = 0
        d.wpacked = self.wpacked.data_ptr()

        def run():
            return self._fn(C.byref(d), st)
        for _ in range(2):
            run()
        for _ in range(rounds * TUNE_REPS):
            rowshift = (self.KH, self.KW, self.stride, self.pad) == (3, 3, 1, 1) and not self.f32 and not self.taps
            for code in XTUNE_CANDIDATES + (XTUNE_ROWSHIFT if rowshift else ()):
                if code % 10 == 3 and self.Cout // self.groups > 64:
                    continue
                if code in (12, 18) and self.Cout // self.groups > 64:
                    continue
                d.tile = code
                if run() == 0:
                    res[code] = min(res.get(code, float("inf")), _time_launches(run, reps))
        d.tile = 0
        return res


class SoftCompGather:

    def __init__(self, weight, bias, channels=128, dtype=torch.bfloat16):
        w = _chk(weight.detach().float().contiguous(), "weight")
        if w.dim() != 2 or w.shape[0] != 49 * channels:
            raise ValueError("SoftComp embedding weight must be [%d, hidden]" % (49 * channels))
        self.C, self.hidden, self.dtype = channels, w.shape[1], dtype
        w4 = w.view(channels, 7, 7, self.hidden)
        self.phases = []
        for py in range(3):
            ky_taps = [6, 3, 0] if py == 0 else [py + 3, py]
            for px in range(3):
                kx_taps = [6, 3, 0] if px == 0 else [px + 3, px]
                wp = w4[:, ky_taps][:, :, kx_taps].permute(0, 3, 1, 2).contiguous()
                layer = PackedConvX(wp, None, [self.hidden], dtype=dtype)
                layer.name = "sc.embedding phase (%d,%d)" % (py, px)
                self.phases.append((py, px, 1 if py == 0 else 0, 1 if px == 0 else 0, layer))
        self.bias = None if bias is None else _chk(bias.detach().float().contiguous(), "bias")
        self._bias_img = {}
        self.tile = 0

    def bias_image(self, fh, fw):
        if self.bias is None:
            return None

        def build():
            rows = self.bias.view(self.C, 49).t().reshape(1, 49 * self.C).expand(fh * fw, 49 * self.C).contiguous()
            return softcomp_fold(rows, 1, fh, fw, 3 * fh, 3 * fw, self.C)[0].contiguous()
        return _lazy(self._bias_img, (fh, fw), "sc.embedding (folded bias image)", build)

    def __call__(self, tokens, out=None, out_dtype=None):
        _chk(tokens, "tokens", self.dtype)
        F_, fh, fw, hid = tokens.shape
        if hid != self.hidden:
            raise ValueError("tokens must be [F, fh, fw, %d]" % self.hidden)
        H, W = 3 * fh, 3 * fw
        if out is None:
            out = torch.empty((F_, H, W, self.C), dtype=out_dtype or self.dtype, device=tokens.device)
        if tuple(out.shape) != (F_, H, W, self.C):
            raise ValueError("out must be [%d,%d,%d,%d]" % (F_, H, W, self.C))
        chunks = list(_image_chunks(F_, fh * fw * hid * tokens.element_size()))
        if len(chunks) > 1:
            for n0, n1 in chunks:
                self(tokens[n0:n1], out=out[n0:n1])
            return out
        bimg = self.bias_image(fh, fw)
        for py, px, pad_y, pad_x, layer in self.phases:
            d = _L.ConvXDesc()
            d.src[0], d.src_ld[0], d.src_coff[0], d.src_cpg[0], d.nsrc = tokens.data_ptr(), hid, 0, hid, 1
            d.N, d.H, d.W, d.Ho, d.Wo = F_, fh, fw, fh, fw
            d.KH, d.KW, d.stride, d.pad = layer.KH, layer.KW, 1, pad_y
            d.groups, d.Cout = 1, self.C
            d.wpacked = layer.wpacked.data_ptr()
            d.dst, d.dst_ld, d.dst_coff, d.dst_dtype = out.data_ptr(), self.C, 0, _dt(out)
            if bimg is not None:
                d.residual, d.res_ld, d.res_coff, d.res_dtype, d.res_bcast = bimg.data_ptr(), self.C, 0, _L.DT_F32, 1
            d.out_grid, d.pad_left = 1, pad_x
            d.out_sy, d.out_sx, d.out_py, d.out_px, d.out_H, d.out_W = 3, 3, py, px, H, W
            d.act, d.slope, d.tile = ACT_NONE, 0.0, self.tile
            if _L.TRACE is not None:
                kc = 32 if layer.f32 else 64
                macs = F_ * fh * fw * self.C * hid * layer.KH * layer.KW
                _L.annotate(layer=layer.name, kernel="conv_%s (gather-form SoftComp)" % ("f32x" if layer.f32 else "f16x" if layer.f16 else "bf16x"),
                            shape="N%d %dx%d %d->%d k%dx%d scatter s3" % (F_, fh, fw, hid, self.C, layer.KH, layer.KW),
                            macs=macs, issued=macs // hid * (-(-hid // kc) * kc))
            _L.check(layer._fn(C.byref(d), _stream()), "conv2d_x (SoftComp phase)")
        return out


class PackedLinearX(PackedConvX):

    def __init__(self, weight, bias, dtype=torch.bfloat16):
        super().__init__(weight, bias, [weight.shape[1]], dtype=dtype)

    def __call__(self, x, out=None, out_dtype=None, residual=None, act=ACT_NONE, slope=0.0, out2=None, tile=0):
        rows = x.numel() // x.shape[-1]
        if out is None:
            out = torch.empty((rows, self.Cout), dtype=out_dtype or self.dtype, device=x.device)
        r4 = None if residual is None else residual.view(rows, 1, 1, residual.shape[-1])
        o2 = None if out2 is None else out2.view(rows, 1, 1, out2.shape[-1])
        super().__call__([x.view(rows, 1, 1, x.shape[-1])], out=out.view(rows, 1, 1, out.shape[-1]), residual=r4, act=act,
                         slope=slope, out2=o2, tile=tile)
        return out


class PackedLinear(PackedConv):

    def __init__(self, weight, bias, bk=None, precision="fp32"):
        super().__init__(weight, bias, [weight.shape[1]], bk=bk, precision=precision)

    def __call__(self, x, out=None, residual=None, act=ACT_NONE, slope=0.0, tile=0, kv_planes=None, out_dtype=None):
        if out_dtype not in (None, torch.float32):
            raise ValueError("PackedLinear writes fp32 results")
        _chk(x, "x")
        rows = x.numel() // x.shape[-1]
        x4 = x.view(rows, 1, 1, x.shape[-1])
        if out is None:
            out = torch.empty((rows, self.Cout), dtype=torch.float32, device=x.device)
        o4 = out.view(rows, 1, 1, out.shape[-1])
        r4 = None if residual is None else residual.view(rows, 1, 1, residual.shape[-1])
        super().__call__([x4], out=o4, residual=r4, act=act, slope=slope, tile=tile, kv_planes=kv_planes)
        return out


class PackedTailConv:

    def __init__(self, weight, bias, dtype=torch.float32):
        lib = _L.load()
        w = _chk(weight.detach().float().contiguous(), "weight")
        self.Cout, self.Cin, self.KH, self.KW = w.shape
        if (self.KH, self.KW) != (3, 3):
            raise ValueError("PackedTailConv: 3x3 kernels only")
        self.dtype = dtype
        if dtype not in _DT_CODE:
            raise TypeError("tensor must be float32, bfloat16 or float16, got %s" % dtype)
        self.wpacked = _pack_weights(lib.e2fgvi_packed_tail_weight_size, lib.e2fgvi_pack_tail_weight, w, dtype, "tail_weight",
                                     self.Cout, self.Cin, extra=(_DT_CODE[dtype],))
        self.bias = None if bias is None else _chk(bias.detach().float().contiguous(), "bias")
        self.name = "conv_tail"

    def __call__(self, sources, out=None, act=ACT_NONE, slope=0.0, out_nchw=True, tile=0):
        x = sources[0] if isinstance(sources, (list, tuple)) else sources
        if not out_nchw:
            raise ValueError("PackedTailConv writes NCHW frames")
        _chk(x, "x", self.dtype)
        N, H, W, ld = x.shape
        if out is None:
            out = torch.empty((N, self.Cout, H, W), dtype=torch.float32, device=x.device)
        _chk(out, "out")
        if tuple(out.shape) != (N, self.Cout, H, W):
            raise ValueError("out shape %s != %s" % (tuple(out.shape), (N, self.Cout, H, W)))
        macs = N * H * W * self.Cout * self.Cin * 9
        tiles = N * -(-H // 16) * -(-W // 32)
        _L.annotate(layer=self.name, kernel="conv_tail", shape="N%d %dx%d %d->%d k3 s1 g1" % (N, H, W, self.Cin, self.Cout),
                    macs=macs, issued=tiles * 640 * 64 * 32)
        _L.check(_L.load().e2fgvi_conv3x3_tail(_ptr(x), _dt(x), ld, _ptr(self.wpacked), _ptr(self.bias), _ptr(out), N, H, W, act,
                                               float(slope), _stream()), "conv3x3_tail")
        return out


_DCN_PACKING = {"fp32": (_L.DT_F32, torch.float32, "mdcn"), "bf16": (_L.DT_BF16, torch.bfloat16, "mdcn_bf16"),
                "fp16": (_L.DT_F16, torch.float16, "mdcn_f16"), "x3": (_L.DT_BF16X3, torch.bfloat16, "mdcn_x3")}


class PackedDcn:
    def __init__(self, weight, bias, deform_groups, stride=1, pad=0, dil=1, mfma="fp32"):
        lib = _L.load()
        if mfma not in _DCN_PACKING:
            raise ValueError("mfma must be 'fp32', 'bf16', 'fp16' or 'x3'")
        self._mfma_dtype, wdtype, self._kernel = _DCN_PACKING[mfma]
        self.mfma_bf16, self.mfma_f16, self.mfma_x3 = mfma == "bf16", mfma == "fp16", mfma == "x3"
        w = _chk(weight.detach().float().contiguous(), "weight")
        self.Cout, self.C, self.KH, self.KW = w.shape
        self.dg, self.stride, self.pad, self.dil = deform_groups, stride, pad, dil
        self.wpacked = _pack_weights(lib.e2fgvi_packed_dcn_weight_size, lib.e2fgvi_pack_dcn_weight, w, wdtype, "dcn_weight",
                                     self._mfma_dtype, self.Cout, self.C, self.KH, self.KW, extra=(deform_groups,))
        self.bias = None if bias is None else _chk(bias.detach().float().contiguous(), "bias")
        self.name = "dcn"

    def __call__(self, sources, offset, mask=None, off_cols=None, flows=None, max_residue=10.0, out=None, tile=0,
                 out_dtype=torch.float32, planar=False):
        lib = _L.load()
        d = _L.MdcnDesc()
        if planar:
            _, N, H, W, _ = sources[0].shape
        else:
            N, H, W, _ = sources[0].shape
        d.src_planar = 1 if planar else 0
        ctot = 0
        for i, t in enumerate(sources):
            _chk_any(t, "source %d" % i)
            if t.dtype != sources[0].dtype:
                raise ValueError("sources must share one dtype")
            c = t.shape[0] * 16 if planar else t.shape[3]
            if planar and (t.dim() != 5 or t.shape[4] != 16 or tuple(t.shape[1:4]) != (N, H, W)):
                raise ValueError("planar source %d must be [C/16, N, H, W, 16]" % i)
            d.src[i], d.src_ld[i], d.src_c[i] = t.data_ptr(), c, c
            ctot += c
        d.src_dtype = _dt(sources[0])
        if ctot != self.C:
            raise ValueError("sources carry %d channels, weight expects %d" % (ctot, self.C))
        d.nsrc = len(sources)
        Ho = (H + 2 * self.pad - (self.dil * (self.KH - 1) + 1)) // self.stride + 1
        Wo = (W + 2 * self.pad - (self.dil * (self.KW - 1) + 1)) // self.stride + 1
        d.N, d.H, d.W, d.Ho, d.Wo = N, H, W, Ho, Wo
        d.KH, d.KW, d.stride, d.pad, d.dil = self.KH, self.KW, self.stride, self.pad, self.dil
        d.deform_groups, d.Cout = self.dg, self.Cout
        K = self.KH * self.KW
        _chk(offset, "offset")
        if tuple(offset.shape[:3]) != (N, Ho, Wo):
            raise ValueError("offset shape %s" % (tuple(offset.shape),))
        d.offset, d.off_ld = offset.data_ptr(), offset.shape[3]
        if mask is None:
            if offset.shape[3] < self.dg * 3 * K:
                raise ValueError("fused offset tensor too narrow")
            d.mask, d.mask_ld = offset.data_ptr() + 4 * self.dg * 2 * K, offset.shape[3]
        else:
            _chk(mask, "mask")
            d.mask, d.mask_ld = mask.data_ptr(), mask.shape[3]
        if flows is not None:
            _chk(flows, "flows")
            if tuple(flows.shape) != (N, Ho, Wo, 4):
                raise ValueError("flows must be [N,Ho,Wo,4]")
            d.flows = flows.data_ptr()
        d.max_residue = max_residue
        d.wpacked = self.wpacked.data_ptr()
        d.bias = self.bias.data_ptr() if self.bias is not None else None
        if out is None:
            out = torch.empty((N, Ho, Wo, self.Cout), dtype=out_dtype, device=sources[0].device)
        _chk_any(out, "out")
        d.dst, d.dst_ld, d.dst_coff, d.tile, d.dst_dtype = out.data_ptr(), out.shape[3], 0, tile, _dt(out)
        d.mfma_dtype = self._mfma_dtype
        if _L.TRACE is not None:
            m = N * Ho * Wo * self.Cout * self.C * K
            _L.annotate(layer=self.name, kernel=self._kernel, shape="N%d %dx%d %d->%d dg%d" % (N, H, W, self.C, self.Cout, self.dg),
                        macs=m, issued=int(m * 6 * 157.3 / 2500.0) if self._mfma_dtype == _L.DT_BF16X3 else m)
        _L.check(lib.e2fgvi_mdcn_nhwc(C.byref(d), _stream()), "mdcn_nhwc")
        return out


def _attn_work(B, T, fh, fw, nkeys):
    qpad = -(-(45 * T) // 32) * 32
    return dict(shape="B%d T%d grid %dx%d" % (B, T, fh, fw), macs=B * (fh // 5) * (fw // 9) * 4 * (45 * T) * (210 * T) * 128 * 2,
                issued=B * 4 * qpad * 128 * 2 * sum(-(-(T * k) // 32) * 32 for k in nkeys.tolist()))


def focal_attention(qkv, kv_pool, key_tab, nkeys, B, T, fh, fw, out=None, waves=0):
    lib = _L.load()
    _chk(qkv, "qkv"); _chk(kv_pool, "kv_pool")
    _chk(key_tab, "key_tab", torch.int32); _chk(nkeys, "nkeys", torch.int32)
    rows = B * T * fh * fw
    if tuple(qkv.shape) != (rows, 1536):
        raise ValueError("qkv must be [%d,1536], got %s" % (rows, tuple(qkv.shape)))
    nwin = (fh // 5) * (fw // 9)
    if tuple(kv_pool.shape) != (B * T * nwin, 1536):
        raise ValueError("kv_pool must be [%d,1536], got %s" % (B * T * nwin, tuple(kv_pool.shape)))
    if key_tab.shape[0] != nwin or nkeys.shape[0] != nwin:
        raise ValueError("key table must have %d rows" % nwin)
    if out is None:
        out = torch.empty((rows, 512), dtype=torch.float32, device=qkv.device)
    _chk(out, "out")
    rpc, ppc = T * fh * fw, T * nwin
    chunks = list(_image_chunks(B, rpc * 1536 * 4))
    if len(chunks) > 1:
        for b0, b1 in chunks:
            focal_attention(qkv[b0 * rpc:b1 * rpc], kv_pool[b0 * ppc:b1 * ppc], key_tab, nkeys, b1 - b0, T, fh, fw,
                            out=out[b0 * rpc:b1 * rpc], waves=waves)
        return out
    if _L.TRACE is not None:
        _L.annotate(layer="attention", kernel="focal_attn", **_attn_work(B, T, fh, fw, nkeys))
    _L.check(lib.e2fgvi_focal_attention(_ptr(qkv), _ptr(kv_pool), _ptr(key_tab), key_tab.shape[1], _ptr(nkeys),
                                        _ptr(out), B, T, fh, fw, waves, _stream()), "focal_attention")
    return out


def split3_kv(rows_1536, out=None):
    lib = _L.load()
    _chk(rows_1536, "qkv rows")
    if rows_1536.dim() != 2 or rows_1536.shape[1] != 1536:
        raise ValueError("split3_kv takes [rows, 1536] fp32 rows")
    rows = rows_1536.shape[0]
    if out is None:
        out = torch.empty((3, rows, 1024), dtype=torch.bfloat16, device=rows_1536.device)
    _chk(out, "planes", torch.bfloat16)
    _L.check(lib.e2fgvi_split3_kv(_ptr(rows_1536), _ptr(out), rows, _stream()), "split3_kv")
    return out


def focal_attention_x3(qkv, planes, key_tab, nkeys, B, T, fh, fw, out=None, waves=0):
    lib = _L.load()
    _chk(qkv, "qkv"); _chk(planes, "planes", torch.bfloat16)
    _chk(key_tab, "key_tab", torch.int32); _chk(nkeys, "nkeys", torch.int32)
    rows = B * T * fh * fw
    nwin = (fh // 5) * (fw // 9)
    if tuple(qkv.shape) != (rows, 1536):
        raise ValueError("qkv must be [%d,1536], got %s" % (rows, tuple(qkv.shape)))
    if tuple(planes.shape) != (3, rows + B * T * nwin, 1024):
        raise ValueError("planes must be [3,%d,1024], got %s" % (rows + B * T * nwin, tuple(planes.shape)))
    if key_tab.shape[0] != nwin or nkeys.shape[0] != nwin:
        raise ValueError("key table must have %d rows" % nwin)
    if out is None:
        out = torch.empty((rows, 512), dtype=torch.float32, device=qkv.device)
    _chk(out, "out")
    if _L.TRACE is not None:
        work = _attn_work(B, T, fh, fw, nkeys)
        work["issued"] = int(work["issued"] * 6 * 157.3 / 2500.0)
        _L.annotate(layer="attention", kernel="focal_attn_x3", **work)
    _L.check(lib.e2fgvi_focal_attention_x3(_ptr(qkv), _ptr(planes), _ptr(key_tab), key_tab.shape[1], _ptr(nkeys), _ptr(out),
                                           B, T, fh, fw, waves, _stream()), "focal_attention_x3")
    return out


def attention_x3_applies(B, T, fh, fw):
    rows = B * T * (fh * fw + (fh // 5) * (fw // 9))
    return (X3_ENABLED and 3 * rows * 2048 < 0xFFFFF000
            and -(-(T * 210) // 32) * 128 + 2 * 49152 + 1280 <= 160 * 1024)


def focal_attention_bf16(qkv, kv_pool, key_tab, nkeys, B, T, fh, fw, out=None, variant=None):
    lib = _L.load()
    if variant is not None:
        prev = lib.e2fgvi_focal_attention_16_variant(int(variant))
        try:
            return focal_attention_bf16(qkv, kv_pool, key_tab, nkeys, B, T, fh, fw, out=out)
        finally:
            lib.e2fgvi_focal_attention_16_variant(prev)
    dt = qkv.dtype if isinstance(qkv, torch.Tensor) and qkv.dtype == torch.float16 else torch.bfloat16
    _chk(qkv, "qkv", dt); _chk(kv_pool, "kv_pool", dt)
    _chk(key_tab, "key_tab", torch.int32); _chk(nkeys, "nkeys", torch.int32)
    rows = B * T * fh * fw
    nwin = (fh // 5) * (fw // 9)
    if tuple(qkv.shape) != (rows, 1536) or tuple(kv_pool.shape) != (B * T * nwin, 1536):
        raise ValueError("qkv must be [%d,1536] and kv_pool [%d,1536]" % (rows, B * T * nwin))
    if key_tab.shape[0] != nwin or nkeys.shape[0] != nwin:
        raise ValueError("key table must have %d rows" % nwin)
    if out is None:
        out = torch.empty((rows, 512), dtype=dt, device=qkv.device)
    _chk(out, "out", dt)
    if _L.TRACE is not None:
        _L.annotate(layer="attention", kernel="focal_attn_f16" if dt == torch.float16 else "focal_attn_bf16",
                    **_attn_work(B, T, fh, fw, nkeys))
    _L.check(lib.e2fgvi_focal_attention_16(_ptr(qkv), _ptr(kv_pool), _ptr(key_tab), key_tab.shape[1], _ptr(nkeys), _ptr(out),
                                           _dt(qkv), B, T, fh, fw, _stream()),
             "focal_attention_f16" if dt == torch.float16 else "focal_attention_bf16")
    return out


def nchw_to_nhwc(x, ld=None, scale=1.0, shift=0.0, out_dtype=torch.float32):
    lib = _L.load()
    _chk(x, "x")
    N, Cc, H, W = x.shape
    ld = Cc if ld is None else ld
    out = torch.empty((N, H, W, ld), dtype=out_dtype, device=x.device)
    _L.check(lib.e2fgvi_nchw_to_nhwc(_ptr(x), _ptr(out), _dt(out), N, Cc, H, W, ld, scale, shift, _stream()), "nchw_to_nhwc")
    return out


def cast(x, dtype):
    lib = _L.load()
    _chk_any(x, "x")
    out = torch.empty(x.shape, dtype=dtype, device=x.device)
    _L.check(lib.e2fgvi_cast(_ptr(x), _dt(x), _ptr(out), _dt(out), x.numel(), _stream()), "cast")
    return out


def nhwc_to_nchw(x, channels=None):
    lib = _L.load()
    _chk(x, "x")
    N, H, W, ld = x.shape
    Cc = ld if channels is None else channels
    out = torch.empty((N, Cc, H, W), dtype=torch.float32, device=x.device)
    _L.check(lib.e2fgvi_nhwc_to_nchw(_ptr(x), ld, _ptr(out), N, Cc, H, W, _stream()), "nhwc_to_nchw")
    return out


def resize_bilinear(x, out_hw, align_corners, src_nchw=False, channels=None, out_ld=None, scale=None, shift=None):
    lib = _L.load()
    if isinstance(x, torch.Tensor) and x.dtype in HALF16:
        _chk(x, "x", x.dtype)
        if src_nchw or scale is not None or shift is not None or channels is not None or out_ld is not None:
            raise ValueError("16-bit resize: plain NHWC -> NHWC only")
        N, H, W, Cc = x.shape
        out = torch.empty((N, out_hw[0], out_hw[1], Cc), dtype=x.dtype, device=x.device)
        _L.check(lib.e2fgvi_resize_bilinear(_ptr(x), _dt(x), 0, Cc, _ptr(out), Cc, N, Cc, H, W, out_hw[0], out_hw[1],
                                            int(align_corners), None, None, _stream()), "resize_bilinear_16")
        return out
    _chk(x, "x")
    if src_nchw:
        N, Cc, H, W = x.shape
        src_ld = 0
    else:
        N, H, W, src_ld = x.shape
        Cc = src_ld if channels is None else channels
    Ho, Wo = out_hw
    out_ld = Cc if out_ld is None else out_ld
    if out_ld > Cc:
        out = torch.zeros((N, Ho, Wo, out_ld), dtype=torch.float32, device=x.device)
    else:
        out = empty_nhwc(N, Ho, Wo, out_ld, x.device)
    for v, nm in ((scale, "scale"), (shift, "shift")):
        if v is not None:
            _chk(v, nm)
            if v.numel() < Cc:
                raise ValueError("%s needs %d entries" % (nm, Cc))
    _L.check(lib.e2fgvi_resize_bilinear(_ptr(x), _L.DT_F32, int(src_nchw), src_ld, _ptr(out), out_ld, N, Cc, H, W, Ho, Wo,
                                        int(align_corners), _ptr(scale), _ptr(shift), _stream()), "resize_bilinear")
    return out


def avgpool2(x):
    lib = _L.load()
    _chk(x, "x")
    N, H, W, Cc = x.shape
    out = empty_nhwc(N, H // 2, W // 2, Cc, x.device)
    _L.check(lib.e2fgvi_avgpool2_nhwc(_ptr(x), _ptr(out), N, H, W, Cc, _stream()), "avgpool2")
    return out


def spynet_level_input(pyr, ref_idx, supp_idx, flow_prev, copy_dtype=None):
    lib = _L.load()
    _chk(pyr, "pyr"); _chk(ref_idx, "ref_idx", torch.int32); _chk(supp_idx, "supp_idx", torch.int32)
    F_, h, w, c = pyr.shape
    if c != 4:
        raise ValueError("pyramid images must be NHWC4")
    Np = ref_idx.numel()
    if flow_prev is not None:
        _chk(flow_prev, "flow_prev")
        if tuple(flow_prev.shape) != (Np, h // 2, w // 2, 2):
            raise ValueError("flow_prev must be [%d,%d,%d,2], got %s" % (Np, h // 2, w // 2, tuple(flow_prev.shape)))
    out = empty_nhwc(Np, h, w, 8, pyr.device)
    if copy_dtype not in (None,) + HALF16:
        raise TypeError("copy_dtype must be None, torch.bfloat16 or torch.float16")
    out16 = torch.empty((Np, h, w, 8), dtype=copy_dtype, device=pyr.device) if copy_dtype is not None else None
    _L.check(lib.e2fgvi_spynet_level_input(_ptr(pyr), _ptr(ref_idx), _ptr(supp_idx), _ptr(flow_prev), _ptr(out), _ptr(out16),
                                           _dt(out16) if out16 is not None else _L.DT_F32, Np, h, w, _stream()),
             "spynet_level_input")
    return (out, out16) if copy_dtype is not None else out


def prop_cond(feat_prop, feat_n2, flow_a, flow_b, flow_img_stride, cond=None, flows=None, cond_dtype=torch.float32,
              flows8=False):
    lib = _L.load()
    _chk_any(feat_prop, "feat_prop")
    N, H, W, Cc = feat_prop.shape
    if cond is None:
        cond = torch.empty((N, H, W, 2 * Cc), dtype=cond_dtype, device=feat_prop.device)
    if flows is None:
        flows = empty_nhwc(N, H, W, 4, feat_prop.device)
    fl8 = (torch.empty((N, H, W, 8), dtype=cond.dtype if cond.dtype == torch.float16 else torch.bfloat16, device=feat_prop.device)
           if flows8 else None)
    f2_ld = 0
    if flow_b is not None:
        _chk(feat_n2, "feat_n2", feat_prop.dtype)
        f2_ld = feat_n2.shape[3]
    _L.check(lib.e2fgvi_prop_cond(_ptr(feat_prop), Cc, _ptr(feat_n2) if flow_b is not None else None, f2_ld, _dt(feat_prop),
                                  C.c_void_p(flow_a.data_ptr()),
                                  C.c_void_p(flow_b.data_ptr()) if flow_b is not None else None,
                                  flow_img_stride, _ptr(cond), _dt(cond), _ptr(flows), _ptr(fl8), N, H, W, Cc, _stream()),
             "prop_cond")
    return (cond, flows, fl8) if flows8 else (cond, flows)


def layernorm(x, gamma, beta, out=None, out_dtype=torch.float32):
    lib = _L.load()
    _chk(x, "x"); _chk(gamma, "gamma"); _chk(beta, "beta")
    Cc = x.shape[-1]
    rows = x.numel() // Cc
    if out is None:
        out = torch.empty(x.shape, dtype=out_dtype, device=x.device)
    _chk_any(out, "out")
    _L.check(lib.e2fgvi_layernorm(_ptr(x), _ptr(gamma), _ptr(beta), _ptr(out), _dt(out), rows, Cc, _stream()), "layernorm")
    return out


def window_pool(x, w45, bias1, BT, fh, fw, out=None):
    lib = _L.load()
    _chk_any(x, "x"); _chk(w45, "w45"); _chk(bias1, "bias1")
    Cc = x.shape[-1]
    rows = BT * (fh // 5) * (fw // 9)
    if out is None:
        out = torch.empty((rows, Cc), dtype=x.dtype, device=x.device)
    elif tuple(_chk(out, "out", x.dtype).shape) != (rows, Cc):
        raise ValueError("window_pool out must be [%d,%d]" % (rows, Cc))
    _L.check(lib.e2fgvi_window_pool(_ptr(x), _dt(x), _ptr(w45), _ptr(bias1), _ptr(out), BT, fh, fw, Cc, _stream()), "window_pool")
    return out


def _ffn_fold(hid, F_, fh, fw, H, W, Cc, gelu):
    lib = _L.load()
    _chk_any(hid, "hid")
    out = torch.empty((F_, H, W, Cc), dtype=hid.dtype, device=hid.device)
    _L.check(lib.e2fgvi_ffn_fold(_ptr(hid), _ptr(out), _dt(hid), gelu, F_, fh, fw, H, W, Cc, _stream()),
             "ffn_fold_gelu" if gelu else "ffn_fold")
    return out


def ffn_fold(hid, F_, fh, fw, H, W, Cc):
    return _ffn_fold(hid, F_, fh, fw, H, W, Cc, 0)


def ffn_fold_gelu(hid, F_, fh, fw, H, W, Cc):
    return _ffn_fold(hid, F_, fh, fw, H, W, Cc, 1)


def _ffn_unfold(folded, fh, fw, out, gelu):
    lib = _L.load()
    _chk_any(folded, "folded")
    F_, H, W, Cc = folded.shape
    if out is None:
        out = torch.empty((F_ * fh * fw, 49 * Cc), dtype=folded.dtype, device=folded.device)
    _chk(out, "out", folded.dtype)
    _L.check(lib.e2fgvi_ffn_unfold(_ptr(folded), _ptr(out), _dt(folded), gelu, F_, fh, fw, H, W, Cc, _stream()),
             "ffn_unfold_gelu" if gelu else "ffn_unfold")
    return out


def ffn_unfold(folded, fh, fw, out=None):
    return _ffn_unfold(folded, fh, fw, out, 0)


def ffn_unfold_gelu(folded, fh, fw, out=None):
    return _ffn_unfold(folded, fh, fw, out, 1)


def to_planar16(x, out=None):
    dt = x.dtype if isinstance(x, torch.Tensor) and x.dtype == torch.float16 else torch.bfloat16
    _chk(x, "x", dt)
    N, H, W, Cc = x.shape
    if out is None:
        out = torch.empty((Cc // 16, N, H, W, 16), dtype=dt, device=x.device)
    _chk(out, "out", dt)
    _L.check(_L.load().e2fgvi_nhwc_to_planar16(_ptr(x), _ptr(out), N * H * W, Cc, _stream()), "nhwc_to_planar16")
    return out


def softcomp_fold(emb, F_, fh, fw, H, W, Cc, bias_hwc=None, residual=None):
    lib = _L.load()
    dt = emb.dtype if isinstance(emb, torch.Tensor) and emb.dtype in HALF16 else torch.float32
    _chk(emb, "emb", dt)
    out = torch.empty((F_, H, W, Cc), dtype=dt, device=emb.device)
    if bias_hwc is not None:
        _chk(bias_hwc, "bias_hwc")
    if residual is not None:
        _chk(residual, "residual", dt)
    _L.check(lib.e2fgvi_softcomp_fold(_ptr(emb), _ptr(bias_hwc), _ptr(residual), _ptr(out), _dt(out), F_, fh, fw, H, W, Cc,
                                      _stream()), "softcomp_fold")
    return out


def _u8(t, name):
    return _chk(t, name, torch.uint8)


def mask_prepare(masks_u8, ytab, xtab, H, W, iterations=4):
    lib = _L.load()
    _u8(masks_u8, "masks")
    _chk(ytab, "ytab", torch.int32); _chk(xtab, "xtab", torch.int32)
    L, Hin, Win = masks_u8.shape
    if ytab.numel() != H or xtab.numel() != W:
        raise ValueError("ytab / xtab must have H / W entries")
    out = torch.empty((L, H, W), dtype=torch.uint8, device=masks_u8.device)
    _L.check(lib.e2fgvi_mask_prepare(_ptr(masks_u8), L, Hin, Win, _ptr(ytab), _ptr(xtab), _ptr(out), H, W, iterations, _stream()),
             "mask_prepare")
    return out


def masked_clip(frames_u8, masks01, ids, Hp, Wp):
    lib = _L.load()
    _u8(frames_u8, "frames"); _u8(masks01, "masks"); _chk(ids, "ids", torch.int32)
    L, H, W, _ = frames_u8.shape
    t = ids.numel()
    out = torch.empty((1, t, 3, Hp, Wp), dtype=torch.float32, device=frames_u8.device)
    _L.check(lib.e2fgvi_masked_clip(_ptr(frames_u8), _ptr(masks01), _ptr(ids), t, H, W, _ptr(out), Hp, Wp, _stream()), "masked_clip")
    return out


def composite(pred, ids, first, frames_u8, masks01, comp):
    lib = _L.load()
    _chk(pred, "pred"); _chk(ids, "ids", torch.int32); _u8(first, "first"); _u8(frames_u8, "frames"); _u8(masks01, "masks")
    _chk(comp, "comp")
    L, H, W, _ = frames_u8.shape
    n = ids.numel()
    if pred.shape[0] < n or pred.shape[1] != 3:
        raise ValueError("pred must hold at least %d frames of 3 channels" % n)
    _L.check(lib.e2fgvi_composite(_ptr(pred), _ptr(ids), _ptr(first), n, _ptr(frames_u8), _ptr(masks01), _ptr(comp), H, W,
                                  pred.shape[2], pred.shape[3], _stream()), "composite")
    return comp


def resample_u8(frames_u8, n_out, axis, bounds, coeffs):
    lib = _L.load()
    _u8(frames_u8, "frames"); _chk(bounds, "bounds", torch.int32); _chk(coeffs, "coeffs", torch.int32)
    if frames_u8.dim() != 4 or frames_u8.shape[3] != 3:
        raise ValueError("frames must be [L,H,W,3], got %s" % (tuple(frames_u8.shape),))
    if axis not in (1, 2):
        raise ValueError("axis must be 1 (H) or 2 (W), got %r" % (axis,))
    if bounds.device != frames_u8.device or coeffs.device != frames_u8.device:
        raise ValueError("frames, bounds and coeffs must be on one device")
    if bounds.dim() != 2 or tuple(bounds.shape) != (n_out, 2) or coeffs.dim() != 2 or coeffs.shape[0] != n_out:
        raise ValueError("bounds must be [n_out,2] and coeffs [n_out,ksize] for n_out = %d" % n_out)
    L, H, W, _ = frames_u8.shape
    n_in = frames_u8.shape[axis]
    ksize = coeffs.shape[1]
    if ksize != 2 * math.ceil(2.0 * max(n_in / n_out, 1.0)) + 1:
        raise ValueError("coeffs of %d taps do not belong to a %d -> %d resize" % (ksize, n_in, n_out))
    shape = (L, n_out, W, 3) if axis == 1 else (L, H, n_out, 3)
    out = torch.empty(shape, dtype=torch.uint8, device=frames_u8.device)
    _L.check(lib.e2fgvi_resample_u8(_ptr(frames_u8), _ptr(out), L, H, W, n_out, axis, _ptr(bounds), _ptr(coeffs), ksize, _stream()),
             "resample_u8")
    return out


def restore_u8(lo, mask_lo, src, ytab, xtab, bx, cx, by, cy, out=None):
    lib = _L.load()
    _u8(lo, "lo"); _u8(mask_lo, "mask_lo"); _u8(src, "src")
    tabs = (("ytab", ytab), ("xtab", xtab), ("bx", bx), ("cx", cx), ("by", by), ("cy", cy))
    for name, t in tabs:
        _chk(t, name, torch.int32)
    if lo.dim() != 4 or lo.shape[3] != 3 or src.dim() != 4 or src.shape[3] != 3 or mask_lo.dim() != 3:
        raise ValueError("lo and src must be [L,.,.,3] and mask_lo [L,.,.], got %s, %s and %s"
                         % (tuple(lo.shape), tuple(src.shape), tuple(mask_lo.shape)))
    L, h, w, _ = lo.shape
    H, W = src.shape[1], src.shape[2]
    if src.shape[0] != L or tuple(mask_lo.shape) != (L, h, w) or min(L, h, w, H, W) < 1:
        raise ValueError("lo %s, mask_lo %s and src %s do not belong to one video" % (tuple(lo.shape), tuple(mask_lo.shape),
                                                                                       tuple(src.shape)))
    if any(t.device != lo.device for t in (mask_lo, src) + tuple(t for _, t in tabs)):
        raise ValueError("lo, mask_lo, src and the tables must be on one device")
    if ytab.dim() != 1 or ytab.numel() != H or xtab.dim() != 1 or xtab.numel() != W:
        raise ValueError("ytab / xtab must have H = %d / W = %d entries" % (H, W))
    for n_in, n_out, b, c, ax in ((w, W, bx, cx, "x"), (h, H, by, cy, "y")):
        if tuple(b.shape) != (n_out, 2) or c.dim() != 2 or c.shape[0] != n_out:
            raise ValueError("b%s must be [%d,2] and c%s [%d,ksize]" % (ax, n_out, ax, n_out))
        if c.shape[1] != 2 * math.ceil(2.0 * max(n_in / n_out, 1.0)) + 1 and not (n_in == n_out and c.shape[1] == 1):
            raise ValueError("c%s of %d taps does not belong to a %d -> %d resize" % (ax, c.shape[1], n_in, n_out))
    if out is None:
        out = torch.empty((L, H, W, 3), dtype=torch.uint8, device=src.device)
    else:
        _u8(out, "out")
        if tuple(out.shape) != (L, H, W, 3) or out.device != src.device:
            raise ValueError("out must be uint8 %s on the device of src" % ((L, H, W, 3),))
    _L.check(lib.e2fgvi_restore_u8(_ptr(lo), _ptr(mask_lo), _ptr(src), _ptr(out), L, h, w, H, W, _ptr(ytab), _ptr(xtab), _ptr(bx),
                                   _ptr(cx), cx.shape[1], _ptr(by), _ptr(cy), cy.shape[1], _stream()), "restore_u8")
    return out


def float_to_u8(x):
    lib = _L.load()
    _chk(x, "x")
    out = torch.empty(x.shape, dtype=torch.uint8, device=x.device)
    _L.check(lib.e2fgvi_float_to_u8(_ptr(x), _ptr(out), x.numel(), _stream()), "float_to_u8")
    return out


def pred_to_u8(pred, H=None, W=None):
    lib = _L.load()
    _chk(pred, "pred")
    N, c, Hp, Wp = pred.shape
    if c != 3:
        raise ValueError("pred must be [N,3,H,W]")
    H, W = H or Hp, W or Wp
    out = torch.empty((N, H, W, 3), dtype=torch.uint8, device=pred.device)
    _L.check(lib.e2fgvi_pred_to_u8(_ptr(pred), _ptr(out), N, H, W, Hp, Wp, _stream()), "pred_to_u8")
    return out


def _slabs(cache, rows, ids, what):
    _chk_any(cache, "cache"); _chk(rows, "rows", cache.dtype); _chk(ids, "ids", torch.int32)
    if cache.dim() < 2 or rows.dim() != cache.dim() or tuple(rows.shape[1:]) != tuple(cache.shape[1:]):
        raise ValueError("%s: cache [slots, ...] and rows [n, ...] must agree past the first dimension, got %s and %s"
                         % (what, tuple(cache.shape), tuple(rows.shape)))
    if ids.dim() != 1 or ids.numel() != rows.shape[0] or rows.shape[0] == 0:
        raise ValueError("%s: ids must be int32 [%d]" % (what, rows.shape[0]))
    if ids.device != cache.device or rows.device != cache.device:
        raise ValueError("%s: cache, rows and ids must be on one device" % what)
    return rows[0].numel() * rows.element_size()


def gather_slabs(cache, ids, out=None):
    lib = _L.load()
    _chk_any(cache, "cache")
    if out is None:
        out = torch.empty((ids.numel(),) + tuple(cache.shape[1:]), dtype=cache.dtype, device=cache.device)
    slab = _slabs(cache, out, ids, "gather_slabs")
    _L.check(lib.e2fgvi_gather_slabs(_ptr(cache), cache.shape[0], _ptr(ids), ids.numel(), slab, _ptr(out), _stream()), "gather_slabs")
    return out


def scatter_slabs(rows, ids, cache):
    lib = _L.load()
    slab = _slabs(cache, rows, ids, "scatter_slabs")
    _L.check(lib.e2fgvi_scatter_slabs(_ptr(rows), _ptr(ids), ids.numel(), slab, _ptr(cache), cache.shape[0], _stream()),
             "scatter_slabs")
    return cache
```

### include/e2fgvi_hip.h

```cpp
#ifndef E2FGVI_HIP_H
#define E2FGVI_HIP_H

#include <stdint.h>

#ifdef __cplusplus
extern "C" {
#endif

#define E2FGVI_EINVAL (-1)
#define E2FGVI_EUNSUP (-2)

#define E2FGVI_ACT_NONE 0
#define E2FGVI_ACT_RELU 1
#define E2FGVI_ACT_LRELU 2
#define E2FGVI_ACT_TANH 3
int e2fgvi_mask_prepare(const uint8_t* masks, int32_t L, int32_t Hin, int32_t Win, const int32_t* ytab, const int32_t* xtab,
                        uint8_t* out, int32_t H, int32_t W, int32_t iterations, void* stream);
int e2fgvi_masked_clip(const uint8_t* frames, const uint8_t* masks, const int32_t* ids, int32_t t, int32_t H, int32_t W,
                       float* clip, int32_t Hp, int32_t Wp, void* stream);
int e2fgvi_composite(const float* pred, const int32_t* ids, const uint8_t* first, int32_t n, const uint8_t* frames,
                     const uint8_t* masks, float* comp, int32_t H, int32_t W, int32_t Hp, int32_t Wp, void* stream);
int e2fgvi_resample_u8(const uint8_t* src, uint8_t* dst, int32_t L, int32_t H, int32_t W, int32_t n_out, int32_t axis,
                       const int32_t* bounds, const int32_t* coeffs, int32_t ksize, void* stream);
int e2fgvi_restore_u8(const uint8_t* lo, const uint8_t* mask_lo, const uint8_t* src, uint8_t* out, int32_t L, int32_t h, int32_t w,
                      int32_t H, int32_t W, const int32_t* ytab, const int32_t* xtab, const int32_t* bounds_x,
                      const int32_t* coeffs_x, int32_t ksize_x, const int32_t* bounds_y, const int32_t* coeffs_y, int32_t ksize_y,
                      void* stream);
int e2fgvi_float_to_u8(const float* src, uint8_t* dst, int64_t n, void* stream);
int e2fgvi_pred_to_u8(const float* pred, uint8_t* dst, int32_t N, int32_t H, int32_t W, int32_t Hp, int32_t Wp, void* stream);
int e2fgvi_gather_slabs(const void* cache, int32_t slots, const int32_t* ids, int32_t n, int64_t slab_bytes, void* window,
                        void* stream);
int e2fgvi_scatter_slabs(const void* rows, const int32_t* ids, int32_t n, int64_t slab_bytes, void* cache, int32_t slots,
                         void* stream);

int64_t e2fgvi_psnr_ssim_workspace(int32_t N, int32_t H, int32_t W);
int e2fgvi_psnr_ssim(const float* img1, const float* img2, int32_t N, int32_t H, int32_t W, int32_t win_size,
                     void* workspace, double* out, void* stream);

#define E2FGVI_ACT_DCNPOST 4

#define E2FGVI_MAX_SRC 4

#define E2FGVI_F32 0
#define E2FGVI_BF16 1
#define E2FGVI_BF16X3 2
#define E2FGVI_F16 3

const char* e2fgvi_last_error(void);
int e2fgvi_abi_version(void);

typedef struct {
    const float* src[E2FGVI_MAX_SRC];
    int32_t src_ld[E2FGVI_MAX_SRC];
    int32_t src_coff[E2FGVI_MAX_SRC];
    int32_t src_cpg[E2FGVI_MAX_SRC];
    int32_t nsrc;
    int32_t N, H, W;
    int32_t Ho, Wo;
    int32_t KH, KW, stride, pad;
    int32_t groups;
    int32_t Cout;
    int32_t bk;
    const float* wpacked;
    const float* bias;
    const float* residual;
    int32_t res_ld, res_coff;
    float* dst;
    int32_t dst_ld, dst_coff;
    int32_t dst_nchw;
    int32_t act;
    float slope;
    int32_t tile;
} e2fgvi_conv_desc;

int e2fgvi_conv2d_nhwc(const e2fgvi_conv_desc* d, void* stream);
int e2fgvi_conv2d_nhwc_nopk(const e2fgvi_conv_desc* d, void* stream);

int64_t e2fgvi_packed_conv_weight_size(int32_t Cout, int32_t groups, int32_t KH, int32_t KW,
                                       int32_t nsrc, const int32_t* src_cpg, int32_t bk);
int e2fgvi_pack_conv_weight(const float* w, float* wpacked, int32_t Cout, int32_t groups,
                            int32_t KH, int32_t KW, int32_t nsrc, const int32_t* src_cpg,
                            int32_t bk, void* stream);

int64_t e2fgvi_packed_winograd_weight_size(int32_t Cout, int32_t groups, int32_t nsrc, const int32_t* src_cpg);
int e2fgvi_pack_winograd_weight(const float* w, float* wpacked, int32_t Cout, int32_t groups, int32_t nsrc,
                                const int32_t* src_cpg, void* stream);
int e2fgvi_conv3x3_winograd(const e2fgvi_conv_desc* d, void* stream);

int64_t e2fgvi_packed_winograd4_weight_size(int32_t Cout, int32_t groups, int32_t nsrc, const int32_t* src_cpg, int32_t fy);
int e2fgvi_pack_winograd4_weight(const float* w, float* wpacked, int32_t Cout, int32_t groups, int32_t nsrc,
                                 const int32_t* src_cpg, int32_t fy, void* stream);
int e2fgvi_conv3x3_winograd4(const e2fgvi_conv_desc* d, int32_t fy, void* stream);

int64_t e2fgvi_packed_tail_weight_size(int32_t Cout, int32_t Cin);
int e2fgvi_pack_tail_weight(const float* w, void* wpacked, int32_t Cout, int32_t Cin, int32_t dtype, void* stream);
int e2fgvi_conv3x3_tail(const void* src, int32_t src_dtype, int32_t src_ld, const void* wpacked, const float* bias, float* dst,
                        int32_t N, int32_t H, int32_t W, int32_t act, float slope, void* stream);

typedef struct {
    const void* src[2];
    int32_t src_ld[2];
    int32_t src_c[2];
    int32_t nsrc;
    int32_t N, H, W, Ho, Wo;
    int32_t KH, KW, stride, pad, dil;
    int32_t deform_groups;
    int32_t Cout;
    const float* offset; int32_t off_ld;
    const float* mask;   int32_t mask_ld;
    const float* flows;
    float max_residue;
    const float* wpacked;
    const float* bias;
    float* dst; int32_t dst_ld, dst_coff;
    int32_t tile;
    int32_t dst_dtype;
    int32_t mfma_dtype;
    int32_t src_dtype;
    int32_t src_planar;
} e2fgvi_mdcn_desc;

int e2fgvi_mdcn_nhwc(const e2fgvi_mdcn_desc* d, void* stream);
int64_t e2fgvi_packed_dcn_weight_size(int32_t mfma_dtype, int32_t Cout, int32_t C, int32_t KH, int32_t KW);
int e2fgvi_pack_dcn_weight(const float* w, void* wpacked, int32_t mfma_dtype, int32_t Cout, int32_t C, int32_t KH, int32_t KW,
                           int32_t deform_groups, void* stream);

int e2fgvi_nhwc_to_planar16(const void* src, void* dst, int64_t P, int32_t C, void* stream);

int e2fgvi_focal_attention(const float* qkv, const float* kv_pool, const int32_t* key_tab,
                           int32_t tab_ld, const int32_t* nkeys, float* out, int32_t B, int32_t T,
                           int32_t fh, int32_t fw, int32_t waves, void* stream);

int e2fgvi_nchw_to_nhwc(const float* src, void* dst, int32_t dst_dtype, int32_t N, int32_t C, int32_t H, int32_t W,
                        int32_t ld, float scale, float shift, void* stream);
int e2fgvi_nhwc_to_nchw(const float* src, int32_t ld, float* dst, int32_t N, int32_t C, int32_t H,
                        int32_t W, void* stream);

int e2fgvi_resize_bilinear(const void* src, int32_t dtype, int32_t src_nchw, int32_t src_ld, void* dst,
                           int32_t dst_ld, int32_t N, int32_t C, int32_t H, int32_t W, int32_t Ho,
                           int32_t Wo, int32_t align_corners, const float* scale,
                           const float* shift, void* stream);

int e2fgvi_avgpool2_nhwc(const float* src, float* dst, int32_t N, int32_t H, int32_t W, int32_t C,
                         void* stream);

int e2fgvi_spynet_level_input(const float* pyr, const int32_t* ref_idx, const int32_t* supp_idx,
                              const float* flow_prev, float* out, void* out16, int32_t out16_dtype, int32_t Np,
                              int32_t h, int32_t w, void* stream);

int e2fgvi_prop_cond(const void* feat_prop, int32_t fp_ld, const void* feat_n2, int32_t f2_ld, int32_t src_dtype,
                     const float* flow_a, const float* flow_b, int64_t flow_img_stride, void* cond, int32_t cond_dtype,
                     float* flows, void* flows8_bf16, int32_t N, int32_t H, int32_t W, int32_t C, void* stream);

int e2fgvi_layernorm(const float* x, const float* gamma, const float* beta, void* y, int32_t y_dtype, int64_t rows,
                     int32_t C, void* stream);

int e2fgvi_window_pool(const void* x, int32_t dtype, const float* w45, const float* bias1, void* pooled,
                       int32_t BT, int32_t fh, int32_t fw, int32_t C, void* stream);

int e2fgvi_ffn_fold(const void* hid, void* folded, int32_t dtype, int32_t gelu, int32_t F, int32_t fh, int32_t fw, int32_t H,
                    int32_t W, int32_t C, void* stream);
int e2fgvi_ffn_unfold(const void* folded, void* out, int32_t dtype, int32_t gelu, int32_t F, int32_t fh, int32_t fw,
                      int32_t H, int32_t W, int32_t C, void* stream);

int e2fgvi_softcomp_fold(const void* emb, const float* bias_hwc, const void* residual,
                         void* dst, int32_t dtype, int32_t F, int32_t fh, int32_t fw, int32_t H, int32_t W,
                         int32_t C, void* stream);
int e2fgvi_cast(const void* src, int32_t src_dtype, void* dst, int32_t dst_dtype, int64_t n, void* stream);

typedef struct {
    const void* src[E2FGVI_MAX_SRC];
    int32_t src_ld[E2FGVI_MAX_SRC];
    int32_t src_coff[E2FGVI_MAX_SRC];
    int32_t src_cpg[E2FGVI_MAX_SRC];
    int32_t nsrc;
    int32_t N, H, W, Ho, Wo;
    int32_t KH, KW, stride, pad;
    int32_t groups;
    int32_t Cout;
    const void* wpacked;
    const float* bias;
    const void* residual;
    int32_t res_ld, res_coff, res_dtype;
    void* dst;
    int32_t dst_ld, dst_coff, dst_dtype;
    void* dst2;
    int32_t dst2_ld, dst2_coff;
    int32_t act;
    float slope;
    int32_t tile;
    int32_t dst_nchw;
    int32_t tap_packed;
    int32_t out_grid, pad_left;
    int32_t out_sy, out_sx, out_py, out_px, out_H, out_W;
    int32_t res_bcast;
    int32_t dst2_split_from;
    int64_t dst2_plane_stride;
} e2fgvi_convx_desc;

int e2fgvi_conv2d_x(const e2fgvi_convx_desc* d, int32_t mode, void* stream);
int64_t e2fgvi_packed_conv_weight_x_size(int32_t mode, int32_t tap_packed, int32_t Cout, int32_t groups, int32_t KH, int32_t KW,
                                         int32_t nsrc, const int32_t* src_cpg);
int e2fgvi_pack_conv_weight_x(const float* w, void* wpacked, int32_t mode, int32_t tap_packed, int32_t Cout, int32_t groups,
                              int32_t KH, int32_t KW, int32_t nsrc, const int32_t* src_cpg, void* stream);

int e2fgvi_conv3x3_winograd_x3(const e2fgvi_conv_desc* d, void* stream);
int64_t e2fgvi_packed_winograd_weight_x3_size(int32_t Cout, int32_t groups, int32_t nsrc, const int32_t* src_cpg);
int e2fgvi_pack_winograd_weight_x3(const float* w, void* wpacked, int32_t Cout, int32_t groups, int32_t nsrc,
                                   const int32_t* src_cpg, void* stream);

int e2fgvi_split3_kv(const float* qkv_rows, void* planes, int64_t rows, void* stream);
int e2fgvi_focal_attention_x3(const float* qkv, const void* planes, const int32_t* key_tab, int32_t tab_ld, const int32_t* nkeys,
                              float* out, int32_t B, int32_t T, int32_t fh, int32_t fw, int32_t waves, void* stream);

int e2fgvi_focal_attention_16(const void* qkv, const void* kv_pool, const int32_t* key_tab, int32_t tab_ld,
                              const int32_t* nkeys, void* out, int32_t dtype, int32_t B, int32_t T, int32_t fh, int32_t fw,
                              void* stream);
int e2fgvi_focal_attention_16_variant(int variant);

#ifdef __cplusplus
}
#endif
#endif
```

Baseline: 967.8 frames/s.

## Add split-bf16 Winograd F(2x4,3x3) x3 conv kernel as a new w3 candidate

Adds a Winograd F(2x4,3x3) convolution kernel that runs on bf16 MFMA with three-way operand splitting, giving fp32-like accuracy. It uses a three-stage LDS DMA pipeline and steady-state plane reloads of the weights, plus host and device weight packing, ISA verifiers, and a new W3 candidate tile (7064) in the ops dispatcher. The aim is fewer MFMA issues per output than the F(2x2) x3 path, because the larger Winograd tile needs 24 rather than 16 transform positions per 4x2 outputs. It adds build complexity and only runs if the tile table or autotuner picks the new candidate.

```diff
diff --git a/e2fgvi_amd/build.py b/e2fgvi_amd/build.py
--- a/e2fgvi_amd/build.py
+++ b/e2fgvi_amd/build.py
@@ -9,11 +9,12 @@
 FLAGS = ["--offload-arch=gfx950", "-O3", "-std=c++17", "-fPIC", "-ffp-contract=fast"]
 NOPK = ["-Xclang", "-target-feature", "-Xclang", "-packed-fp32-ops"]
 UNITS = [("error.hip", "error.o", []), ("conv.hip", "conv.o", []), ("conv.hip", "conv_nopk.o", NOPK + ["-DE2_NOPK_VARIANT"]),
-         ("conv_bf16x.hip", "conv_bf16x.o", NOPK), ("conv_wino.hip", "conv_wino.o", NOPK), ("conv_wino.hip", "conv_wino_x3.o", NOPK + ["-DE2_WINO_X3=1"]), ("conv_wino4.hip", "conv_wino4.o", NOPK), ("conv_tail.hip", "conv_tail.o", NOPK),
+         ("conv_bf16x.hip", "conv_bf16x.o", NOPK), ("conv_wino.hip", "conv_wino.o", NOPK), ("conv_wino.hip", "conv_wino_x3.o", NOPK + ["-DE2_WINO_X3=1"]), ("conv_wino4.hip", "conv_wino4.o", NOPK),
+         ("conv_wino4.hip", "conv_wino4_x3.o", NOPK + ["-DE2_WINO4_X3=1"]), ("conv_tail.hip", "conv_tail.o", NOPK),
          ("mdcn.hip", "mdcn.o", NOPK), ("attention.hip", "attention.o", []),
          ("attention_bf16.hip", "attention_bf16.o", NOPK), ("attention_x3.hip", "attention_x3.o", NOPK), ("misc.hip", "misc.o", NOPK),
          ("video.hip", "video.o", NOPK), ("metrics.hip", "metrics.o", NOPK)]
-NOPK_OBJECTS = ("conv_nopk.o", "conv_bf16x.o", "conv_wino.o", "conv_wino4.o", "conv_wino_x3.o", "conv_tail.o", "mdcn.o", "attention_bf16.o", "attention_x3.o", "misc.o", "video.o", "metrics.o")
+NOPK_OBJECTS = ("conv_nopk.o", "conv_bf16x.o", "conv_wino.o", "conv_wino4.o", "conv_wino_x3.o", "conv_wino4_x3.o", "conv_tail.o", "mdcn.o", "attention_bf16.o", "attention_x3.o", "misc.o", "video.o", "metrics.o")
 OBJDUMP = "/opt/rocm/lib/llvm/bin/llvm-objdump"
 
 
@@ -61,6 +62,7 @@
             verify_wino_waits(objdir)
             verify_exit_reuse(objdir)
             verify_no_scratch(objdir)
+            verify_no_scratch(objdir, "conv_wino4_x3.o", "conv_wino_x3f_kernel")
     return out
 
 
@@ -165,12 +167,38 @@
                 spans.append((addr_to_idx[tgt], i))
     loops = 0
     rolling = "conv_wino_x3w_kernel" in name
+    steady = "conv_wino_x3f_kernel" in name
     for lo, hi in spans:
         inner = [m for m in marks if lo <= m <= hi]
         if not inner or any(lo <= l2 and h2 <= hi and (l2, h2) != (lo, hi) and any(l2 <= m <= h2 for m in inner)
                             for l2, h2 in spans):
             continue
         loops += 1
+        if steady:
+            total = sum(1 for k in range(lo, hi + 1) if vmem.match(ins[k][1]))
+            for j, m in enumerate(inner):
+                rng = range(m + 2, inner[j + 1]) if j + 1 < len(inner) else list(range(m + 2, hi + 1)) + list(range(lo, inner[0]))
+                grp, first = [], None
+                for k in rng:
+                    if not vmem.match(ins[k][1]):
+                        continue
+                    if ins[k][1] != "buffer_load_dwordx4" or " lds" in ins[k][2]:
+                        break
+                    grp.append(k)
+                n = int(re.search(r"vmcnt\((\d+)\)", ins[m][2]).group(1))
+                if not grp or n != total - len(grp):
+                    raise RuntimeError("%s: %s: explicit s_waitcnt vmcnt(%d) at 0x%x: the trip issues %d vector-memory instructions, "
+                                       "%d of them the plane loads behind this wait" % (obj, name[:60], n, ins[m][0], total, len(grp)))
+                dest, breg = set(), set()
+                for k in grp:
+                    dest |= _vregs(ins[k][2].split(",")[0])
+                for k in range(m + 2, grp[0]):
+                    if "mfma" in ins[k][1]:
+                        breg |= _vregs([x.strip() for x in ins[k][2].split(",")][2])
+                if dest != breg:
+                    raise RuntimeError("%s: %s: the plane loads behind the wait at 0x%x do not reload exactly the B operands of the "
+                                       "MFMAs in front of them" % (obj, name[:60], ins[m][0]))
+            continue
         if rolling:
             counts = [int(re.search(r"vmcnt\((\d+)\)", ins[m][2]).group(1)) for m in inner]
             for a, b in zip(inner, inner[1:]):
@@ -199,7 +227,7 @@
     return loops
 
 
-def verify_wino_waits(objdir=None, objects=("conv_wino.o", "conv_wino_x3.o", "conv_wino4.o")):
+def verify_wino_waits(objdir=None, objects=("conv_wino.o", "conv_wino_x3.o", "conv_wino4.o", "conv_wino4_x3.o")):
     objdir = objdir or os.path.join(CSRC, "build")
     if not os.path.exists(OBJDUMP):
         return 0
@@ -343,7 +371,7 @@
     return edges
 
 
-EXIT_REUSE_OBJECTS = ("conv_wino.o", "conv_wino_x3.o", "conv_wino4.o")
+EXIT_REUSE_OBJECTS = ("conv_wino.o", "conv_wino_x3.o", "conv_wino4.o", "conv_wino4_x3.o")
 
 
 def verify_exit_reuse(objdir=None, objects=EXIT_REUSE_OBJECTS):
diff --git a/e2fgvi_amd/csrc/conv_wino4.hip b/e2fgvi_amd/csrc/conv_wino4.hip
--- a/e2fgvi_amd/csrc/conv_wino4.hip
+++ b/e2fgvi_amd/csrc/conv_wino4.hip
@@ -1,5 +1,9 @@
 #include "common.h"
 #include <utility>
+
+#ifndef E2_WINO4_X3
+#define E2_WINO4_X3 0
+#endif
 
 #ifndef E2_CLAIM_AFTER_LOOP
 #define E2_CLAIM_AFTER_LOOP(r) asm volatile("" : "+v"(r))
@@ -453,6 +457,7 @@
     return true;
 }
 
+#if !E2_WINO4_X3
 __global__ void pack_wino4_weight_kernel(const float* __restrict__ w, float* __restrict__ wp, const W4Pack p) {
     const long long idx = (long long)blockIdx.x * blockDim.x + threadIdx.x;
     if (idx >= p.total) return;
@@ -498,8 +503,419 @@
     return 0;
 }
 
-}
-
+#endif
+
+#if E2_WINO4_X3
+
+typedef __bf16 w4_bf16x8 __attribute__((ext_vector_type(8)));
+typedef unsigned int w4_u32x4 __attribute__((ext_vector_type(4)));
+typedef __attribute__((address_space(3))) void w4_lds_void;
+
+__device__ __forceinline__ void w4_split4(const f32x4& v, unsigned (&H)[2], unsigned (&M)[2], unsigned (&L)[2]) {
+    float x[4];
+#pragma unroll
+    for (int j = 0; j < 4; ++j) x[j] = v[j];
+#pragma unroll
+    for (int j = 0; j < 2; ++j) e2_split2(x[2 * j], x[2 * j + 1], H[j], M[j], L[j]);
+}
+
+__device__ __forceinline__ void w4_dma_piece(w4_i32x4 rsrc, unsigned lds_dst, unsigned voff) {
+    unsigned keep;
+    asm volatile("s_mov_b32 %0, m0\n\ts_mov_b32 m0, %3\n\ts_nop 2\n\tbuffer_load_dwordx4 %1, %2, 0 offen lds\n\ts_mov_b32 m0, %0"
+                 : "=&s"(keep) : "v"(voff), "s"(rsrc), "s"(lds_dst) : "memory");
+}
+
+template <int BN>
+__global__ __launch_bounds__(512, 2) void conv_wino_x3f_kernel(const W4Params p) {
+    constexpr int SC = 2;
+    constexpr int TN = BN / 32;
+    constexpr int NPOS = 24;
+    constexpr int RAW_H = 18;
+    constexpr int PLANE_ROW = 6;
+    constexpr int PLANE_RAW = RAW_H * PLANE_ROW * 16;
+    constexpr int PLANE_BYTES = PLANE_RAW + ((16 - PLANE_RAW % 128) + 128) % 128;
+    constexpr int CHUNK_USED = 8 * PLANE_BYTES;
+    constexpr int CHUNK_BYTES = (CHUNK_USED + 1023) / 1024 * 1024;
+    constexpr int STAGE_BYTES = SC * CHUNK_BYTES;
+    constexpr int NSTAGE = 3;
+    constexpr int EPI_BYTES = NPOS * 32 * 32 * 4;
+    constexpr int SMEM = (NSTAGE * STAGE_BYTES > EPI_BYTES) ? NSTAGE * STAGE_BYTES : EPI_BYTES;
+    constexpr int PIECES = CHUNK_BYTES / 1024;
+    constexpr int NPMAX = (PIECES + 7) / 8;
+    static_assert(PIECES > 8 && PIECES <= 16, "every wave has one or two pieces per chunk");
+
+    __shared__ __attribute__((aligned(1024))) unsigned char smem[SMEM];
+
+    const int tid = threadIdx.x;
+    const int lane = tid & 63, wave = tid >> 6;
+    const int g = blockIdx.y;
+    const int logical = xcd_remap(blockIdx.x, p.nblk);
+    const int mblocks = p.N * p.blocksY * p.blocksX;
+    const int tile_n = logical / mblocks;
+    int rem = logical - tile_n * mblocks;
+    const int img = rem / (p.blocksY * p.blocksX);
+    rem -= img * (p.blocksY * p.blocksX);
+    const int by = rem / p.blocksX, bx = rem - by * p.blocksX;
+    const int n0 = tile_n * BN;
+    const int y0 = by * 16 - 1, x0 = bx * 16 - 1;
+
+    unsigned dma_pix[NPMAX];
+    {
+        constexpr int UP = PLANE_BYTES / 16;
+#pragma unroll
+        for (int j = 0; j < NPMAX; ++j) {
+            const int U = (wave + 8 * j) * 64 + lane;
+            const int plane = U / UP, r2 = U - plane * UP;
+            const int py = r2 / PLANE_ROW, c = r2 - py * PLANE_ROW;
+            const int pxx = 4 * c + (plane & 3);
+            const int gy_ = y0 + py, gx_ = x0 + pxx;
+            const bool in = plane < 8 && py < RAW_H && pxx < W4_RAW_W && gy_ >= 0 && gy_ < p.H && gx_ >= 0 && gx_ < p.W;
+            dma_pix[j] = in ? ((unsigned)((img * p.H + gy_) * p.W + gx_) | ((unsigned)(plane >> 2) << 30)) : W4_OOB;
+        }
+    }
+    const unsigned smem_lds = (unsigned)(unsigned long long)(w4_lds_void*)smem;
+    int w_s = 0, w_c0 = 0;
+    const float* w_src = p.src[0];
+    unsigned w_bytes = p.src_bytes[0], w_ld4 = (unsigned)p.ld[0] * 4u, w_chan = (unsigned)(p.coff[0] + g * p.cpg[0]) * 4u;
+    int w_cpg = p.cpg[0];
+    int w_left = p.nchunks;
+    auto dma_chunk = [&](auto W_, auto NPW_, unsigned lds_chunk) __attribute__((always_inline)) {
+        constexpr int WV = decltype(W_)::value, NPW = decltype(NPW_)::value;
+        const w4_i32x4 rs = w4_rsrc_words(w_src, w_bytes);
+        const unsigned chan = w_chan + (unsigned)w_c0 * 4u;
+        const bool half = w_c0 + 4 >= w_cpg;
+        const bool live = w_left-- > 0;
+#pragma unroll
+        for (int j = 0; j < NPW; ++j) {
+            const unsigned pix = dma_pix[j] & 0x3FFFFFFFu, kq = (dma_pix[j] >> 30) & 1u;
+            unsigned off = (live && (int)dma_pix[j] >= 0 && !(half && kq)) ? pix * w_ld4 + chan + kq * 16u : W4_OOB;
+            asm volatile("" : "+v"(off));
+            w4_dma_piece(rs, __builtin_amdgcn_readfirstlane(lds_chunk + (unsigned)((WV + 8 * j) * 1024)), off);
+        }
+        w_c0 += 8;
+        if (w_c0 >= w_cpg) {
+            w_c0 = 0;
+            ++w_s;
+            if (w_s == p.nsrc) w_s = 0;
+            if (p.nsrc > 1) {
+#define E2_WALK_ARM(S) { w_src = p.src[S]; w_bytes = p.src_bytes[S]; w_ld4 = (unsigned)p.ld[S] * 4u; \
+                         w_chan = (unsigned)(p.coff[S] + g * p.cpg[S]) * 4u; w_cpg = p.cpg[S]; }
+                if (w_s == 0) E2_WALK_ARM(0) else if (w_s == 1) E2_WALK_ARM(1) else if (w_s == 2) E2_WALK_ARM(2) else E2_WALK_ARM(3)
+#undef E2_WALK_ARM
+            }
+        }
+    };
+
+    const int i = lane & 31, h = lane >> 5;
+    const int ty = i >> 2, tx = i & 3;
+    const int a_lane = h * CHUNK_BYTES + (2 * ty * PLANE_ROW + tx) * 16;
+
+    const w4_i32x4 wrsrc = w4_rsrc_words(reinterpret_cast<const char*>(p.w) + (long long)g * p.wgroup_bytes, p.wgroup_bytes);
+    const unsigned u_step = (unsigned)(NPOS * 6) * (unsigned)p.Npad * 16u;
+    const unsigned u_plane = 2u * (unsigned)p.Npad * 16u;
+    unsigned u_lane = (unsigned)((h * p.Npad + n0 + i) * 16);
+    auto load_plane = [&](f32x4& v, unsigned soff) __attribute__((always_inline)) {
+        asm volatile("s_nop 4\n\tbuffer_load_dwordx4 %0, %1, %2, %3 offen" : "=v"(v) : "v"(u_lane), "s"(wrsrc), "s"(soff) : "memory");
+    };
+    f32x4 bw[3][TN][3];
+    f32x16 acc[3][TN];
+#pragma unroll
+    for (int a = 0; a < 3; ++a)
+#pragma unroll
+        for (int n = 0; n < TN; ++n)
+#pragma unroll
+            for (int r = 0; r < 16; ++r) acc[a][n][r] = 0.f;
+
+    const int nstages = (p.nchunks + SC - 1) / SC;
+
+    auto k_loop = [&](auto XI_, auto HF_) __attribute__((always_inline)) {
+        constexpr int XI = decltype(XI_)::value;
+        constexpr int HF = decltype(HF_)::value;
+        constexpr int R0 = (XI == 0) ? 0 : 1, R1 = (XI == 3) ? 3 : 2;
+        constexpr int WV = 2 * XI + HF;
+        constexpr int NPW = (PIECES - WV + 7) / 8;
+        const unsigned u_pos = (unsigned)((XI * 6 + 3 * HF) * 6) * (unsigned)p.Npad * 16u;
+        unsigned u_n[TN];
+#pragma unroll
+        for (int n = 0; n < TN; ++n) u_n[n] = (n0 + n * 32 < p.Npad) ? (unsigned)(n * 32 * 16) : 0u;
+        auto load_planes = [&](int a) __attribute__((always_inline)) {
+#pragma unroll
+            for (int n = 0; n < TN; ++n)
+#pragma unroll
+                for (int pl = 0; pl < 3; ++pl)
+                    load_plane(bw[a][n][pl], u_pos + (unsigned)(a * 3 + pl) * u_plane + u_n[n]);
+        };
+#pragma unroll
+        for (int c4 = 0; c4 < 2 * SC; ++c4)
+            dma_chunk(IC4<WV>{}, IC4<NPW>{}, smem_lds + (unsigned)((c4 / SC) * STAGE_BYTES + (c4 % SC) * CHUNK_BYTES));
+#pragma unroll
+        for (int a = 0; a < 3; ++a) load_planes(a);
+        u_lane += u_step;
+        asm volatile("s_waitcnt vmcnt(0)" ::: "memory");
+        __syncthreads();
+
+        auto col_comb = [&](const f32x4 (&e)[5], auto A_) -> f32x4 {
+            constexpr int nu = 3 * HF + decltype(A_)::value;
+            bool first = true;
+            f32x4 acc_v = {0.f, 0.f, 0.f, 0.f};
+#pragma unroll
+            for (int j = 0; j < 5; ++j) {
+                const float c = bt4(nu, HF + j);
+                if (c == 0.f) continue;
+                acc_v = first ? c * e[j] : acc_v + c * e[j];
+                first = false;
+            }
+            return acc_v;
+        };
+        auto prep = [&](const unsigned char* rm, w4_bf16x8 (&A)[9]) __attribute__((always_inline)) {
+            unsigned P[9][4];
+#pragma unroll
+            for (int kq = 0; kq < 2; ++kq) {
+                f32x4 e[5];
+#pragma unroll
+                for (int j = 0; j < 5; ++j) {
+                    const int col = HF + j;
+                    const int off = (kq * 4 + (col & 3)) * PLANE_BYTES + (col >> 2) * 16;
+                    const f32x4 d0 = *reinterpret_cast<const f32x4*>(rm + off + R0 * PLANE_ROW * 16);
+                    const f32x4 d1 = *reinterpret_cast<const f32x4*>(rm + off + R1 * PLANE_ROW * 16);
+                    e[j] = XI == 1 ? d0 + d1 : XI == 2 ? d1 - d0 : d0 - d1;
+                }
+                w4_static_for<3>([&](auto A_) {
+                    constexpr int a = decltype(A_)::value;
+                    const f32x4 v = col_comb(e, A_);
+                    unsigned H[2], M[2], L[2];
+                    w4_split4(v, H, M, L);
+                    P[3 * a][2 * kq] = H[0]; P[3 * a][2 * kq + 1] = H[1];
+                    P[3 * a + 1][2 * kq] = M[0]; P[3 * a + 1][2 * kq + 1] = M[1];
+                    P[3 * a + 2][2 * kq] = L[0]; P[3 * a + 2][2 * kq + 1] = L[1];
+                });
+            }
+#pragma unroll
+            for (int f = 0; f < 9; ++f) {
+                w4_u32x4 t = {P[f][0], P[f][1], P[f][2], P[f][3]};
+                A[f] = __builtin_bit_cast(w4_bf16x8, t);
+            }
+        };
+        auto mma = [&](const w4_bf16x8 (&A)[9]) __attribute__((always_inline)) {
+#pragma unroll
+            for (int a = 0; a < 3; ++a) {
+                asm volatile("s_waitcnt vmcnt(%0)\n\ts_waitcnt vmcnt(%0)" ::"n"(SC * NPW + 6 * TN) : "memory");
+#pragma unroll
+                for (int n = 0; n < TN; ++n)
+#pragma unroll
+                    for (int pl = 0; pl < 3; ++pl) asm volatile("" : "+v"(bw[a][n][pl]));
+                __builtin_amdgcn_sched_barrier(0);
+                const w4_bf16x8 xh = A[3 * a], xm = A[3 * a + 1], xl = A[3 * a + 2];
+                w4_bf16x8 uh[TN], um[TN], ul[TN];
+#pragma unroll
+                for (int n = 0; n < TN; ++n) {
+                    uh[n] = __builtin_bit_cast(w4_bf16x8, bw[a][n][0]);
+                    um[n] = __builtin_bit_cast(w4_bf16x8, bw[a][n][1]);
+                    ul[n] = __builtin_bit_cast(w4_bf16x8, bw[a][n][2]);
+                }
+#pragma unroll
+                for (int n = 0; n < TN; ++n) acc[a][n] = __builtin_amdgcn_mfma_f32_32x32x16_bf16(xl, uh[n], acc[a][n], 0, 0, 0);
+#pragma unroll
+                for (int n = 0; n < TN; ++n) acc[a][n] = __builtin_amdgcn_mfma_f32_32x32x16_bf16(xh, ul[n], acc[a][n], 0, 0, 0);
+#pragma unroll
+                for (int n = 0; n < TN; ++n) acc[a][n] = __builtin_amdgcn_mfma_f32_32x32x16_bf16(xm, um[n], acc[a][n], 0, 0, 0);
+#pragma unroll
+                for (int n = 0; n < TN; ++n) acc[a][n] = __builtin_amdgcn_mfma_f32_32x32x16_bf16(xm, uh[n], acc[a][n], 0, 0, 0);
+#pragma unroll
+                for (int n = 0; n < TN; ++n) acc[a][n] = __builtin_amdgcn_mfma_f32_32x32x16_bf16(xh, um[n], acc[a][n], 0, 0, 0);
+#pragma unroll
+                for (int n = 0; n < TN; ++n) acc[a][n] = __builtin_amdgcn_mfma_f32_32x32x16_bf16(xh, uh[n], acc[a][n], 0, 0, 0);
+                __builtin_amdgcn_sched_barrier(0);
+                load_planes(a);
+                __builtin_amdgcn_sched_barrier(0);
+            }
+        };
+        int slot = 0;
+        for (int st = 0; st < nstages; ++st) {
+            const unsigned char* rm = smem + slot * STAGE_BYTES + a_lane;
+            const unsigned ahead = smem_lds + (unsigned)((slot == 0 ? 2 : slot - 1) * STAGE_BYTES);
+#pragma unroll
+            for (int q = 0; q < SC; ++q) dma_chunk(IC4<WV>{}, IC4<NPW>{}, ahead + (unsigned)(q * CHUNK_BYTES));
+            __builtin_amdgcn_sched_barrier(0);
+            w4_bf16x8 A[9];
+            prep(rm, A);
+            __builtin_amdgcn_sched_barrier(0);
+            mma(A);
+            u_lane += u_step;
+            slot = slot == 2 ? 0 : slot + 1;
+            __syncthreads();
+        }
+    };
+    switch (wave) {
+        case 0: k_loop(IC4<0>{}, IC4<0>{}); break;
+        case 1: k_loop(IC4<0>{}, IC4<1>{}); break;
+        case 2: k_loop(IC4<1>{}, IC4<0>{}); break;
+        case 3: k_loop(IC4<1>{}, IC4<1>{}); break;
+        case 4: k_loop(IC4<2>{}, IC4<0>{}); break;
+        case 5: k_loop(IC4<2>{}, IC4<1>{}); break;
+        case 6: k_loop(IC4<3>{}, IC4<0>{}); break;
+        default: k_loop(IC4<3>{}, IC4<1>{}); break;
+    }
+    asm volatile("s_waitcnt vmcnt(0)" ::: "memory");
+#pragma unroll
+    for (int a = 0; a < 3; ++a)
+#pragma unroll
+        for (int n = 0; n < TN; ++n)
+#pragma unroll
+            for (int pl = 0; pl < 3; ++pl) E2_CLAIM_AFTER_LOOP(bw[a][n][pl]);
+    __syncthreads();
+
+    float* E = reinterpret_cast<float*>(smem);
+    const int HW = p.H * p.W;
+    const int pos0 = (wave >> 1) * 6 + 3 * (wave & 1);
+#pragma unroll
+    for (int nh = 0; nh < TN; ++nh) {
+        if (nh) __syncthreads();
+#pragma unroll
+        for (int a = 0; a < 3; ++a)
+#pragma unroll
+            for (int r = 0; r < 16; ++r) {
+                const int tile = (r & 3) + 8 * (r >> 2) + 4 * h;
+                E[((pos0 + a) * 32 + tile) * 32 + i] = acc[a][nh][r];
+            }
+        __syncthreads();
+        const int cq = tid & 7, tile = (tid >> 3) & 31, oy = tid >> 8;
+        const int n = n0 + nh * 32 + cq * 4;
+        const int oyy = by * 16 + 2 * (tile >> 2) + oy, oxx = bx * 16 + 4 * (tile & 3);
+        if (n < p.Cout_g && oyy < p.H && oxx < p.W) {
+            f32x4 sc[6];
+            const float* Ey = E + ((oy * 6) * 32 + tile) * 32 + cq * 4;
+#pragma unroll
+            for (int nu = 0; nu < 6; ++nu) {
+                const f32x4 m0 = *reinterpret_cast<const f32x4*>(Ey + (0 * 6 + nu) * 1024);
+                const f32x4 m1 = *reinterpret_cast<const f32x4*>(Ey + (1 * 6 + nu) * 1024);
+                const f32x4 m2 = *reinterpret_cast<const f32x4*>(Ey + (2 * 6 + nu) * 1024);
+                sc[nu] = oy ? m0 - m1 - m2 : m0 + m1 + m2;
+            }
+            f32x4 y[4];
+#pragma unroll
+            for (int ox = 0; ox < 4; ++ox) {
+                bool first = true;
+                f32x4 a4 = {0.f, 0.f, 0.f, 0.f};
+#pragma unroll
+                for (int nu = 0; nu < 6; ++nu) {
+                    const float c = at4(ox, nu);
+                    if (c == 0.f) continue;
+                    a4 = first ? c * sc[nu] : a4 + c * sc[nu];
+                    first = false;
+                }
+                y[ox] = a4;
+            }
+            const int co = g * p.Cout_g + n;
+            const long long pix0 = (long long)img * HW + (long long)oyy * p.W + oxx;
+            const bool full = n + 3 < p.Cout_g;
+            f32x4 bv = {0.f, 0.f, 0.f, 0.f};
+            if (p.bias) {
+#pragma unroll
+                for (int c = 0; c < 4; ++c) bv[c] = (full || n + c < p.Cout_g) ? p.bias[co + c] : 0.f;
+            }
+#pragma unroll
+            for (int px = 0; px < 4; ++px) {
+                if (oxx + px >= p.W) break;
+                const long long pix = pix0 + px;
+                f32x4 v = y[px] + bv;
+                if (p.act == E2FGVI_ACT_DCNPOST) {
+                    const f32x4 fl = *reinterpret_cast<const f32x4*>(p.res + pix * 4);
+                    const float flv[4] = {fl[0], fl[1], fl[2], fl[3]};
+#pragma unroll
+                    for (int c = 0; c < 4; ++c) v[c] = w4_dcn_post(v[c], co + c, p.Cout, flv, p.slope);
+                } else {
+                    if (p.res) {
+                        const float* r = p.res + pix * p.res_ld + p.res_coff + co;
+                        if (p.vec_store && full) v = v + *reinterpret_cast<const f32x4*>(r);
+                        else {
+#pragma unroll
+                            for (int c = 0; c < 4; ++c) if (full || n + c < p.Cout_g) v[c] += r[c];
+                        }
+                    }
+#pragma unroll
+                    for (int c = 0; c < 4; ++c) v[c] = w4_act(v[c], p.act, p.slope);
+                }
+                float* o = p.dst + pix * p.dst_ld + p.dst_coff + co;
+                if (p.vec_store && full) *reinterpret_cast<f32x4*>(o) = v;
+                else {
+#pragma unroll
+                    for (int c = 0; c < 4; ++c) if (full || n + c < p.Cout_g) o[c] = v[c];
+                }
+            }
+        }
+    }
+}
+
+__host__ __device__ inline float w4_u_x3(const float* f, int a) {
+    const int xi = a / 6, nu = a - xi * 6;
+    float acc = 0.f;
+    for (int r = 0; r < 3; ++r) {
+        float row = 0.f;
+        for (int c = 0; c < 3; ++c) row = __builtin_fmaf(f[r * 3 + c], g4(nu, c), row);
+        acc = __builtin_fmaf(g2(xi, r), row, acc);
+    }
+    return acc;
+}
+__host__ __device__ inline void w4_split3(float v, unsigned short (&o)[3]) {
+#pragma clang fp contract(off)
+    const unsigned xb = __builtin_bit_cast(unsigned, v);
+    const float r = v - __builtin_bit_cast(float, xb & 0xFFFF0000u);
+    const unsigned rb = __builtin_bit_cast(unsigned, r);
+    const float r2 = r - __builtin_bit_cast(float, rb & 0xFFFF0000u);
+    o[0] = (unsigned short)(xb >> 16);
+    o[1] = (unsigned short)(rb >> 16);
+    o[2] = (unsigned short)(__builtin_bit_cast(unsigned, r2) >> 16);
+}
+
+__global__ void pack_wino4_weight_x3_kernel(const float* __restrict__ w, unsigned short* __restrict__ wp, const W4Pack p, int nstages) {
+    const long long per_group = (long long)nstages * 24 * 2 * p.Npad * 8;
+    const long long idx = (long long)blockIdx.x * blockDim.x + threadIdx.x;
+    if (idx >= per_group * p.groups) return;
+    const int g = (int)(idx / per_group);
+    long long rem = idx - (long long)g * per_group;
+    const int j = (int)(rem & 7);
+    rem >>= 3;
+    const int n = (int)(rem % p.Npad);
+    rem /= p.Npad;
+    const int h = (int)(rem & 1);
+    rem >>= 1;
+    const int a = (int)(rem % 24);
+    const int stage = (int)(rem / 24);
+    const int chunk = 2 * stage + h;
+    float v = 0.f;
+    if (chunk < p.nchunks && n < p.Cout_g) {
+        int s = 0, prefix = 0, lc = chunk;
+        while (lc >= (p.cpg[s] + 7) / 8) { lc -= (p.cpg[s] + 7) / 8; prefix += p.cpg[s]; ++s; }
+        const int ch = lc * 8 + j;
+        if (ch < p.cpg[s]) v = w4_u_x3(w + ((long long)(g * p.Cout_g + n) * p.Cin_g + prefix + ch) * 9, a);
+    }
+    unsigned short pc[3];
+    w4_split3(v, pc);
+    const long long plane = 2LL * p.Npad * 8;
+    unsigned short* o = wp + (long long)g * per_group * 3 + ((long long)(stage * 24 + a) * 3) * plane + ((long long)h * p.Npad + n) * 8 + j;
+    o[0] = pc[0];
+    o[plane] = pc[1];
+    o[2 * plane] = pc[2];
+}
+
+template <int BN>
+int launch_wino_x3f(W4Params& p, int groups, hipStream_t st) {
+    p.blocksY = cdiv(p.H, 16);
+    p.blocksX = cdiv(p.W, 16);
+    p.tilesN = cdiv(p.Cout_g, BN);
+    const long long nblk = (long long)p.N * p.blocksY * p.blocksX * p.tilesN;
+    E2_REQUIRE(nblk < 2147483647LL, E2FGVI_EUNSUP, "conv3x3_winograd4_x3: grid too large");
+    p.nblk = (int)nblk;
+    hipLaunchKernelGGL((conv_wino_x3f_kernel<BN>), dim3(p.nblk, groups, 1), dim3(512), 0, st, p);
+    E2_LAUNCH_CHECK("conv3x3_winograd4_x3");
+    return 0;
+}
+#endif
+
+}
+
+#if !E2_WINO4_X3
 extern "C" int64_t e2fgvi_packed_winograd4_weight_size(int32_t Cout, int32_t groups, int32_t nsrc, const int32_t* src_cpg,
                                                        int32_t fy) {
     W4Pack q;
@@ -521,14 +937,16 @@
     return 0;
 }
 
-extern "C" int e2fgvi_conv3x3_winograd4(const e2fgvi_conv_desc* d, int32_t fy, void* stream) {
+#endif
+
+static int w4_run(const e2fgvi_conv_desc* d, int32_t fy, void* stream, bool x3) {
     E2_REQUIRE(d, E2FGVI_EINVAL, "conv3x3_winograd4: null descriptor");
     W4Pack q;
     E2_REQUIRE(w4_geometry(d->Cout, d->groups, d->nsrc, d->src_cpg, fy, &q), E2FGVI_EINVAL,
                "conv3x3_winograd4: bad geometry (channels per source must be multiples of 4, fy = 2)");
     E2_REQUIRE(d->KH == 3 && d->KW == 3 && d->stride == 1 && d->pad == 1, E2FGVI_EUNSUP,
                "conv3x3_winograd4: only 3x3, stride 1, pad 1");
-    E2_REQUIRE(d->N > 0 && d->H > 0 && d->W > 0 && d->H % fy == 0 && d->W % 4 == 0, E2FGVI_EUNSUP,
+    E2_REQUIRE(d->N > 0 && d->H > 0 && d->W > 0 && (x3 || (d->H % fy == 0 && d->W % 4 == 0)), E2FGVI_EUNSUP,
                "conv3x3_winograd4: H must be a multiple of fy and W a multiple of 4");
     E2_REQUIRE(d->Ho == d->H && d->Wo == d->W, E2FGVI_EINVAL, "conv3x3_winograd4: Ho/Wo must equal H/W");
     E2_REQUIRE(d->wpacked && d->dst, E2FGVI_EINVAL, "conv3x3_winograd4: null weight/dst");
@@ -550,13 +968,14 @@
         p.src[s] = d->src[s]; p.ld[s] = d->src_ld[s]; p.coff[s] = d->src_coff[s]; p.cpg[s] = d->src_cpg[s];
         p.src_bytes[s] = (unsigned)bytes;
     }
-    E2_REQUIRE(q.wgroup_elems * 4 < 0x70000000LL, E2FGVI_EUNSUP, "conv3x3_winograd4: packed weight group >= 1.75 GiB");
+    E2_REQUIRE(q.wgroup_elems * 4 * (x3 ? 2 : 1) < 0x70000000LL, E2FGVI_EUNSUP, "conv3x3_winograd4: packed weight group >= 1.75 GiB");
     E2_REQUIRE(((uintptr_t)d->wpacked & 15) == 0, E2FGVI_EINVAL, "conv3x3_winograd4: packed weight not 16-byte aligned");
     p.nsrc = d->nsrc;
     p.N = d->N; p.H = d->H; p.W = d->W;
     p.Cout = d->Cout; p.Cout_g = q.Cout_g; p.Npad = q.Npad;
     p.nchunks = q.nchunks;
     p.wgroup_elems = q.wgroup_elems; p.wgroup_bytes = (unsigned)(q.wgroup_elems * 4);
+    if (x3) p.wgroup_bytes = (unsigned)((long long)((q.nchunks + 1) / 2) * q.npos * 3 * 2 * q.Npad * 16);
     p.w = (const float*)d->wpacked; p.bias = d->bias;
     p.res = d->residual; p.res_ld = d->res_ld; p.res_coff = d->res_coff;
     p.dst = d->dst; p.dst_ld = d->dst_ld; p.dst_coff = d->dst_coff;
@@ -568,7 +987,54 @@
     hipStream_t st = (hipStream_t)stream;
     int tile = d->tile;
     if (!tile) tile = 64;
+#if E2_WINO4_X3
+    if (fy == 2 && tile == 64) return launch_wino_x3f<64>(p, d->groups, st);
+    e2fgvi_set_error("conv3x3_winograd4_x3: tile must be 0 (auto) or 64 couts per workgroup");
+#else
+    (void)x3;
     if (fy == 2 && tile == 64) return launch_wino4<2, 64>(p, d->groups, st);
     e2fgvi_set_error("conv3x3_winograd4: fy must be 2 and tile 0 (auto) or 64 couts per workgroup (the other shapes were pruned in round 6)");
+#endif
     return E2FGVI_EUNSUP;
 }
+
+#if E2_WINO4_X3
+extern "C" int64_t e2fgvi_packed_winograd4_weight_x3_size(int32_t Cout, int32_t groups, int32_t nsrc, const int32_t* src_cpg) {
+    W4Pack q;
+    if (!src_cpg || !w4_geometry(Cout, groups, nsrc, src_cpg, 2, &q)) {
+        e2fgvi_set_error("packed_winograd4_weight_x3_size: bad geometry (channels per source must be multiples of 4)");
+        return E2FGVI_EINVAL;
+    }
+    return (long long)((q.nchunks + 1) / 2) * q.npos * 3 * 2 * q.Npad * 8 * groups;
+}
+
+extern "C" int e2fgvi_pack_winograd4_weight_x3(const float* w, void* wpacked, int32_t Cout, int32_t groups, int32_t nsrc,
+                                               const int32_t* src_cpg, void* stream) {
+    W4Pack q;
+    E2_REQUIRE(w && wpacked && src_cpg, E2FGVI_EINVAL, "pack_winograd4_weight_x3: null pointer");
+    E2_REQUIRE(w4_geometry(Cout, groups, nsrc, src_cpg, 2, &q), E2FGVI_EINVAL, "pack_winograd4_weight_x3: bad geometry");
+    const int nstages = (q.nchunks + 1) / 2;
+    const long long values = (long long)nstages * q.npos * 2 * q.Npad * 8 * groups;
+    hipLaunchKernelGGL(pack_wino4_weight_x3_kernel, dim3((unsigned)cdiv64(values, 256)), dim3(256), 0, (hipStream_t)stream, w,
+                       (unsigned short*)wpacked, q, nstages);
+    E2_LAUNCH_CHECK("pack_winograd4_weight_x3");
+    return 0;
+}
+
+extern "C" int e2fgvi_winograd4_weight_x3_host(const float* w, int64_t nfilters, float* u, uint16_t* planes) {
+    E2_REQUIRE(w && u && planes && nfilters >= 0, E2FGVI_EINVAL, "winograd4_weight_x3_host: null pointer");
+    for (int64_t f = 0; f < nfilters; ++f)
+        for (int a = 0; a < 24; ++a) {
+            const float v = w4_u_x3(w + f * 9, a);
+            unsigned short pc[3];
+            w4_split3(v, pc);
+            u[f * 24 + a] = v;
+            for (int pl = 0; pl < 3; ++pl) planes[((int64_t)pl * nfilters + f) * 24 + a] = pc[pl];
+        }
+    return 0;
+}
+
+extern "C" int e2fgvi_conv3x3_winograd4_x3(const e2fgvi_conv_desc* d, void* stream) { return w4_run(d, 2, stream, true); }
+#else
+extern "C" int e2fgvi_conv3x3_winograd4(const e2fgvi_conv_desc* d, int32_t fy, void* stream) { return w4_run(d, fy, stream, false); }
+#endif
diff --git a/e2fgvi_amd/lib.py b/e2fgvi_amd/lib.py
--- a/e2fgvi_amd/lib.py
+++ b/e2fgvi_amd/lib.py
@@ -81,6 +81,10 @@
     "e2fgvi_packed_winograd4_weight_size": (_i64, [_i32, _i32, _i32, C.POINTER(_i32), _i32]),
     "e2fgvi_pack_winograd4_weight": (C.c_int, [_fp, _fp, _i32, _i32, _i32, C.POINTER(_i32), _i32, _fp]),
     "e2fgvi_conv3x3_winograd4": (C.c_int, [C.POINTER(ConvDesc), _i32, _fp]),
+    "e2fgvi_packed_winograd4_weight_x3_size": (_i64, [_i32, _i32, _i32, C.POINTER(_i32)]),
+    "e2fgvi_pack_winograd4_weight_x3": (C.c_int, [_fp, _fp, _i32, _i32, _i32, C.POINTER(_i32), _fp]),
+    "e2fgvi_winograd4_weight_x3_host": (C.c_int, [_fp, _i64, _fp, _fp]),
+    "e2fgvi_conv3x3_winograd4_x3": (C.c_int, [C.POINTER(ConvDesc), _fp]),
     "e2fgvi_packed_tail_weight_size": (_i64, [_i32, _i32]),
     "e2fgvi_pack_tail_weight": (C.c_int, [_fp, _fp, _i32, _i32, _i32, _fp]),
     "e2fgvi_conv3x3_tail": (C.c_int, [_fp, _i32, _i32, _fp, _fp, _fp, _i32, _i32, _i32, _i32, C.c_float, _fp]),
@@ -134,6 +138,8 @@
     if m:
         fy = int(m.group(1))
         f = (fy + 2) * 6 / (fy * 4 * 9.0)
+    elif k.startswith("conv_wino_x3f"):
+        f = 24 / 72.0
     elif k.startswith("conv_wino"):
         f = 16 / 36.0
     if "x3" in k:
diff --git a/e2fgvi_amd/ops.py b/e2fgvi_amd/ops.py
--- a/e2fgvi_amd/ops.py
+++ b/e2fgvi_amd/ops.py
@@ -42,8 +42,9 @@
 X3_MARGIN = 0.97
 X3_BASE = 30000
 W3_BASE = 40000
-W3_CANDIDATES = (132, 164, 32, 5132, 6064)
+W3_CANDIDATES = (132, 164, 32, 5132, 6064, 7064)
 W3_WIDE = 6064
+W3_F24 = 7064
 W3_WIDE_FALLBACK = 164
 DMA_BASE = 2000
 
@@ -388,6 +389,13 @@
                                  torch.bfloat16, "winograd_weight_x3", *self._wgeom())
         return _lazy(vars(self), "_w3", self.name + " (split-operand Winograd weights)", build)
 
+    def _wino_x3f(self):
+        def build():
+            lib = _L.load()
+            return _pack_weights(lib.e2fgvi_packed_winograd4_weight_x3_size, lib.e2fgvi_pack_winograd4_weight_x3, self._w_oihw,
+                                 torch.bfloat16, "winograd4_weight_x3", *self._wgeom())
+        return _lazy(self._w4, "x3", self.name + " (split-operand Winograd F(2x4,3x3) weights)", build)
+
     def _alt3(self):
         if any(c % 4 for c in self.cpg):
             return self.alt3
@@ -404,6 +412,12 @@
             cin_p = sum(-(-c // 8) * 8 for c in self.cpg)
             issued = pix * (-(-cout_g // bn) * bn) * self.groups * cin_p * (fy + 2) * 6 // (fy * 4)
             kern = "conv_wino4<F(%dx4),%d>" % (fy, bn)
+        elif family == "w3" and tile == W3_F24:
+            asked = W3_BASE + tile
+            pix = N * (-(-H // 16) * 16) * (-(-W // 16) * 16)
+            cin_p = -(-sum(-(-c // 8) for c in self.cpg) // 2) * 16
+            issued = int(pix * (-(-cout_g // 64) * 64) * self.groups * cin_p * 3 * _L.X3_PIPE)
+            kern = "conv_wino_x3f<64>"
         elif family == "w3":
             asked = W3_BASE + tile
             shape = tile % 1000
@@ -536,6 +550,9 @@
 
     def _run(self, d, family, tile, use_wino):
         lib, st = _L.load(), _stream()
+        if family == "w3" and tile == W3_F24:
+            d.tile, d.wpacked = 64, self._wino_x3f().data_ptr()
+            return lib.e2fgvi_conv3x3_winograd4_x3(C.byref(d), st), "conv3x3_winograd4_x3"
         if family == "w3":
             d.tile, d.wpacked = tile, self._wino_x3().data_ptr()
             return lib.e2fgvi_conv3x3_winograd_x3(C.byref(d), st), "conv3x3_winograd_x3"
@@ -562,7 +579,7 @@
             if family == "dma":
                 self._alt()(srcs, tile=tile, **kw)
                 return False
-            if family == "x3" or (family == "w3" and self._wino_x3() is None):
+            if family == "x3" or (family == "w3" and self._w_oihw is None):
                 family, tile = plan.static
         except _L.HipError:
             if not plan.from_table:
diff --git a/include/e2fgvi_hip.h b/include/e2fgvi_hip.h
--- a/include/e2fgvi_hip.h
+++ b/include/e2fgvi_hip.h
@@ -91,6 +91,11 @@
 int e2fgvi_pack_winograd4_weight(const float* w, float* wpacked, int32_t Cout, int32_t groups, int32_t nsrc,
                                  const int32_t* src_cpg, int32_t fy, void* stream);
 int e2fgvi_conv3x3_winograd4(const e2fgvi_conv_desc* d, int32_t fy, void* stream);
+int64_t e2fgvi_packed_winograd4_weight_x3_size(int32_t Cout, int32_t groups, int32_t nsrc, const int32_t* src_cpg);
+int e2fgvi_pack_winograd4_weight_x3(const float* w, void* wpacked, int32_t Cout, int32_t groups, int32_t nsrc,
+                                    const int32_t* src_cpg, void* stream);
+int e2fgvi_winograd4_weight_x3_host(const float* w, int64_t nfilters, float* u, uint16_t* planes);
+int e2fgvi_conv3x3_winograd4_x3(const e2fgvi_conv_desc* d, void* stream);
 
 int64_t e2fgvi_packed_tail_weight_size(int32_t Cout, int32_t Cin);
 int e2fgvi_pack_tail_weight(const float* w, void* wpacked, int32_t Cout, int32_t Cin, int32_t dtype, void* stream);
```

After: 931.3 frames/s. 3.8% lower.
